# bytedance/DecompDiff

Measured on AMD Instinct MI355X. Metric: denoising steps/sec (1000-step reverse) per pocket, higher is better.
Workload: dtype f32

## Files before the change

### decompdiff_amd/csrc/dd_api.hip

```cpp
#include <mutex>
#include <thread>
#include <vector>
#include <stdlib.h>
#include <string.h>
#include <stdio.h>
#include <string>
#include <sys/stat.h>
#include <unistd.h>

#include "dd_kernels.hpp"

namespace dd {

struct Workspace {
  float *xa, *xb, *h, *hb, *ew, *P, *PL, *PB, *P2, *PL2, *PB2, *Ek, *Ev, *Rk, *Rv, *q1bl, *qn, *ql, *ql2, *qlnb, *qb, *A, *Anb, *dxe, *dxb, *ga, *gc, *gr, *h2, *hs;
  int32_t* nbr;
  int32_t* counters;
  size_t total;
};

static inline size_t align64(size_t n) { return (n + 63) & ~(size_t)63; }

static Workspace carve(float* base, int B, int NP, int NL, int K) {
  Workspace w;
  const size_t N = (size_t)NP + NL, Eb = (size_t)NL * (NL > 0 ? NL - 1 : 0);
  size_t off = 0;
  auto take = [&](size_t n) { float* p = base ? base + off : nullptr; off += align64(n); return p; };
  w.xa = take(B * N * 3);
  w.xb = take(B * N * 3);
  w.h = take(B * N * 128);
  w.hb = take(B * Eb * 128);
  w.nbr = reinterpret_cast<int32_t*>(take(B * N * K));
  w.ew = take(B * N * K);
  w.P = take(B * N * 640);
  w.PL = take((size_t)B * NL * 1280);
  w.PB = take(B * Eb * 640);
  w.P2 = take(B * N * 256);
  w.PL2 = take((size_t)B * NL * 1024);
  w.PB2 = take(B * Eb * 256);
  w.Ek = take(B * Eb * 128);
  w.Ev = take(B * Eb * 128);
  w.Rk = take(B * Eb * 128);
  w.Rv = take(B * Eb * 128);
  w.q1bl = take(B * Eb * 128);
  w.qn = take(B * N * 128);
  w.ql = take((size_t)B * NL * 128);
  w.ql2 = take((size_t)B * NL * 128);
  w.qlnb = take((size_t)B * NL * 128);
  w.qb = take(B * Eb * 128);
  w.A = take(B * N * 128);
  w.Anb = take((size_t)B * NL * 128);
  w.dxe = take((size_t)B * NL * 3);
  w.dxb = take((size_t)B * NL * 3);
  w.ga = take((size_t)B * NL * 3);
  w.gc = take((size_t)B * NL * 3);
  w.gr = take((size_t)B * NL * 3);
#if defined(DD_DEBUG_OPTIONS) && DD_DEBUG_OPTIONS
  w.h2 = take(B * N * 128);
  w.hs = take(B * N * 128);
#else
  w.h2 = w.hs = nullptr;
#endif
  w.counters = reinterpret_cast<int32_t*>(take(DD_NUM_COUNTERS + DD_NUM_FLAGS));
  w.total = off;
  return w;
}

static inline int num_v(const dd_sampler* s) { return s->num_v > 0 ? s->num_v : DD_NUM_V; }

static int check_shapes(const dd_sampler* s) {
  if (!s || !s->weights || !s->slot_off || !s->workspace) return DD_ERR_BAD_ARG;
  if (s->B <= 0 || s->NP < 0 || s->NL < 2 || s->K <= 0 || s->num_layers < 1 || s->num_layers > 64) return DD_ERR_BAD_ARG;
  const int N = s->NP + s->NL;
  if (s->NL > DD_NL_MAX || N > DD_N_MAX || s->K > DD_KNN_MAX || s->K > N - 1) return DD_ERR_UNSUPPORTED_SHAPE;
  if (s->num_v != 0 && s->num_v != 8 && s->num_v != 13 && s->num_v != 23) return DD_ERR_UNSUPPORTED_SHAPE;
  if (num_v(s) != DD_NUM_V && s->l0_tables != nullptr) return DD_ERR_BAD_ARG;
  if (s->workspace_floats < dd_workspace_floats(s->B, s->NP, s->NL, s->K)) return DD_ERR_WORKSPACE_TOO_SMALL;
  if ((s->nl_real != nullptr) != (s->bl_prefix != nullptr) || (s->np_real != nullptr && s->nl_real == nullptr)) return DD_ERR_BAD_ARG;
  return DD_OK;
}

struct Profiler {
  static constexpr int MAXEV = 512;
  hipEvent_t start[MAXEV], stop[MAXEV];
  int cat[MAXEV];
  int n = 0, created = 0;
};
static Profiler* g_prof = nullptr;

struct ProfScope {
  hipStream_t st; int idx;
  ProfScope(int cat, hipStream_t s) : st(s), idx(-1) {
    if (g_prof && g_prof->n < Profiler::MAXEV) {
      idx = g_prof->n++;
      g_prof->cat[idx] = cat;
      (void)hipEventRecord(g_prof->start[idx], st);
    }
  }
  ~ProfScope() { if (idx >= 0) (void)hipEventRecord(g_prof->stop[idx], st); }
};
#define DD_TRYP(cat, expr)               \
  do {                                  \
    ProfScope prof_scope__(cat, st);    \
    int rc__ = (expr);                  \
    if (rc__ != DD_OK) return rc__;     \
  } while (0)

#define DD_TRY(expr)            \
  do {                          \
    int rc__ = (expr);          \
    if (rc__ != DD_OK) return rc__; \
  } while (0)

extern int g_gemm_ksplit;
#if defined(DD_DEBUG_OPTIONS) && DD_DEBUG_OPTIONS
extern int g_tail_variant;
#endif
static bool g_gemm_ksplit_on() { return g_gemm_ksplit != 0; }
struct DevCtx {
  hipStream_t side = nullptr;
  hipEvent_t ev_qa_fork[8], ev_qb_fork[8], ev_fork[9], ev_join[9];
};
static DevCtx g_dev_ctx[16];
static std::mutex g_capture_mutex;
static DevCtx& dev_ctx() {
  int dev = 0;
  if (hipGetDevice(&dev) != hipSuccess || dev < 0 || dev >= 16) dev = 0;
  return g_dev_ctx[dev];
}
#define g_side (dev_ctx().side)
#define g_ev_qa_fork (dev_ctx().ev_qa_fork)
#define g_ev_qb_fork (dev_ctx().ev_qb_fork)
#define g_ev_fork (dev_ctx().ev_fork)
#define g_ev_join (dev_ctx().ev_join)
#ifndef DD_SIDE_LIN_DEFAULT
#define DD_SIDE_LIN_DEFAULT 0
#endif
#if defined(DD_DEBUG_OPTIONS) && DD_DEBUG_OPTIONS
#define DD_OPT static int
#else
#define DD_OPT static constexpr int
#endif
DD_OPT g_step_fused = 1;
DD_OPT g_step_fold = 1;
DD_OPT g_xup_in_asm = 1;
DD_OPT g_sched = 4;
DD_OPT g_xup_in_pos = 0;
DD_OPT g_fused_max_nl = DD_NL_MAX;
DD_OPT g_defer_pos = 0;
DD_OPT g_lin_with_pb2 = 1;
DD_OPT g_pb_early = 1;
DD_OPT g_q1_in_gemm = 1;
DD_OPT g_l0_tables = 1;
DD_OPT g_head_fused = 1;
DD_OPT g_side_lin = DD_SIDE_LIN_DEFAULT;
static int g_lin_in_node = [] { const char* e = getenv("DD_LIN_IN_NODE"); return e ? (e[0] == '1' ? 1 : (e[0] == '0' ? 0 : -1)) : -1; }();
static int g_lin_proj_main = [] { const char* e = getenv("DD_LIN_PROJ_MAIN"); return e ? (e[0] == '1' ? 1 : 0) : 0; }();
static bool lin_in_node_for(int B, int NL) {
  if (g_lin_in_node >= 0) return g_lin_in_node != 0;
  return (long)B * NL * (NL - 1) < 8L * 256 * 2;
}
DD_OPT g_head_rows_first = 0;
DD_OPT g_heads_early = 1;
DD_OPT g_q_in_pos = 1;
extern int g_pos_waves;
DD_OPT g_p2_in_pos = 0;
static int g_side_low_priority = [] { const char* e = getenv("DD_SIDE_PRIO"); return (e && e[0] == '1') ? 1 : ((e && e[0] == '2') ? 2 : 0); }();
static int g_overlap = 1;
static int ensure_side_stream() {
  if (g_side) return DD_OK;
  {
    int lo = 0, hi = 0;
    if (hipDeviceGetStreamPriorityRange(&lo, &hi) != hipSuccess) { lo = 0; (void)hipGetLastError(); }
    if (hipStreamCreateWithPriority(&g_side, hipStreamNonBlocking, g_side_low_priority == 1 ? lo : (g_side_low_priority == 2 ? hi : 0)) != hipSuccess) return DD_ERR_HIP;
  }
  for (int i = 0; i < 8; ++i)
    if (hipEventCreateWithFlags(&g_ev_qa_fork[i], hipEventDisableTiming) != hipSuccess ||
        hipEventCreateWithFlags(&g_ev_qb_fork[i], hipEventDisableTiming) != hipSuccess)
      return DD_ERR_HIP;
  for (int i = 0; i < 9; ++i)
    if (hipEventCreateWithFlags(&g_ev_fork[i], hipEventDisableTiming) != hipSuccess ||
        hipEventCreateWithFlags(&g_ev_join[i], hipEventDisableTiming) != hipSuccess)
      return DD_ERR_HIP;
  return DD_OK;
}

static int g_fuse = 1;
extern long long* g_gemm_dbg;
extern long long* g_node_trace;
static long long* g_dbg_clock = nullptr;
static int g_dbg_mode = -1;


static int attn_dispatch(int mode, const AttnArgs& a0, hipStream_t st) {
  AttnArgs a = a0;
  a.dbg_clock = (mode == g_dbg_mode) ? g_dbg_clock : nullptr;
  return launch_attn2(mode, a, st);
}

struct StepFold {
  bool advance = false;
  bool fold_tail = false;
  const float* xprev = nullptr;
};

__global__ __launch_bounds__(256) void k_bond_head_pre_att(const float* __restrict__ P, const float* __restrict__ x,
                                                           const float* __restrict__ dxe, const float* __restrict__ dxb, int NP, int NL,
                                                           const float* __restrict__ W_r, const float* __restrict__ b1,
                                                           const float* __restrict__ offset, float coeff,
                                                           const int32_t* __restrict__ nl_real, long rows, float* __restrict__ out) {
  constexpr int G = 20;
  const int lane = threadIdx.x & 63;
  const long nwaves = (long)gridDim.x * 4;
  float2 wr[G];
  float c[G];
#pragma unroll
  for (int k = 0; k < G; ++k) {
    wr[k] = *reinterpret_cast<const float2*>(W_r + k * 128 + 2 * lane);
    c[k] = offset[k];
  }
  const float2 bb = *reinterpret_cast<const float2*>(b1 + 2 * lane);
  const int N = NP + NL, NLm1 = NL - 1;
  const long Eb = (long)NL * NLm1;
  for (long e = (long)blockIdx.x * 4 + (threadIdx.x >> 6); e < rows; e += nwaves) {
    const int b = (int)(e / Eb);
    const int r = (int)(e - (long)b * Eb);
    const int t = r / NLm1, sp = r - t * NLm1;
    const int src = sp + (sp >= t);
    float2* o = reinterpret_cast<float2*>(out + e * 128 + 2 * lane);
    if (nl_real != nullptr && (t >= nl_real[b] || src >= nl_real[b])) {
      *o = make_float2(0.f, 0.f);
      continue;
    }
    float xd[3], xs[3];
#pragma unroll
    for (int q = 0; q < 3; ++q) {
      xd[q] = x[((long)b * N + NP + t) * 3 + q];
      xs[q] = x[((long)b * N + NP + src) * 3 + q];
      if (dxe != nullptr) {
        const long id = ((long)b * NL + t) * 3 + q, is = ((long)b * NL + src) * 3 + q;
// ... 208 lines not shown
      pe.B = B; pe.NP = NP; pe.NL = NL; pe.K = K; pe.x = xcur; pe.nbr = w.nbr; pe.ew = w.ew;
      pe.kd = w.PL2; pe.vd = w.PL2 + 128; pe.ld_kd = pe.ld_vd = 1024; pe.ks = w.P2; pe.vs = w.P2 + 128; pe.ld_ks = pe.ld_vs = 256;
      pe.q = w.ql; pe.Akp = LW(l, DD_PE_Akp); pe.Avp = LW(l, DD_PE_Avp); pe.lnk = LW(l, DD_PE_lnk); pe.lnv = LW(l, DD_PE_lnv);
      pe.W2k = LW(l, DD_PE_W2k); pe.W2v16 = LW(l, DD_PE_W2v); pe.b2v16 = LW(l, DD_PE_b2v); pe.out = w.dxe;
      pb.B = B; pb.NP = NP; pb.NL = NL; pb.K = K; pb.x = xcur;
      pb.kd = w.PL2 + 384; pb.ks = w.PL2 + 512; pb.vd = w.PL2 + 640; pb.vs = w.PL2 + 768; pb.ld_kd = pb.ld_ks = pb.ld_vd = pb.ld_vs = 1024;
      pb.ke = w.PB2; pb.ve = w.PB2 + 128; pb.ld_ke = pb.ld_ve = 256;
      pb.q = w.ql2; pb.lnk = LW(l, DD_PB_lnk); pb.lnv = LW(l, DD_PB_lnv);
      pb.W2k = LW(l, DD_PB_W2k); pb.W2v16 = LW(l, DD_PB_W2v); pb.b2v16 = LW(l, DD_PB_b2v); pb.out = w.dxb; pb.x_next = nullptr;
      pe.qhid = w.PL2 + 256; pe.ld_qhid = 1024; pe.lnq = LW(l, DD_PE_lnq); pe.W2q = LW(l, DD_PE_W2qT); pe.b2q = LW(l, DD_PE_b2q);
      pb.qhid = w.PL2 + 896; pb.ld_qhid = 1024; pb.lnq = LW(l, DD_PB_lnq); pb.W2q = LW(l, DD_PB_W2qT); pb.b2q = LW(l, DD_PB_b2q);
      if (two_streams) {
        if (hipEventRecord(g_ev_fork[l], st) != hipSuccess) return DD_ERR_HIP;
        DD_TRY(launch_gemm_tail(ta, st));
        if (hipStreamWaitEvent(g_side, g_ev_fork[l], 0) != hipSuccess) return DD_ERR_HIP;
        DD_TRY(launch_gemm_tail(tb, g_side));
        if (l + 1 == L && hipEventRecord(g_ev_join[l], g_side) != hipSuccess) return DD_ERR_HIP;
        DD_TRY(launch_attn2_pos(pe, pb, st));
      } else {
        DD_TRYP(DD_PROF_GEMM, launch_gemm_tail(ta, st));
        DD_TRYP(DD_PROF_GEMM, launch_gemm_tail(tb, st));
        DD_TRYP(DD_PROF_ATTN_PE, launch_attn2_pos(pe, pb, st));
      }
      if (l + 1 < L && ta.total + tb.total != total_mid) return DD_ERR_BAD_ARG;
      const bool deferred = l + 1 < L || (fold && fold->fold_tail);
      if (deferred) xup_prev = xcur;
      else DD_TRYP(DD_PROF_MISC, launch_xupdate(xcur, w.dxe, w.dxb, B, NP, NL, xnext, st));
    }
    float* t = xcur; xcur = xnext; xnext = t;
  }
  if (head_join && hipStreamWaitEvent(st, g_ev_join[8], 0) != hipSuccess) return DD_ERR_HIP;
  if (two_streams && hipStreamWaitEvent(st, g_ev_join[L - 1], 0) != hipSuccess) return DD_ERR_HIP;
  if (!s->pred_pos) return DD_ERR_BAD_ARG;
  if (xup_prev != nullptr) {
    fold->xprev = xup_prev;
    return DD_OK;
  }
  DD_TRYP(DD_PROF_MISC, launch_extract_ligand(xcur, B, NP, NL, s->pred_pos, st));
  return DD_OK;
}

#endif

static int check_node_out(const dd_node_out* no, const dd_sampler* s) {
  if (no == nullptr) return DD_OK;
  if (!s || no->num_layers != s->num_layers || no->num_layers < 1 || no->num_layers > 64) return DD_ERR_BAD_ARG;
  for (int l = 0; l < no->num_layers; ++l)
    if (!no->layer[l] || (reinterpret_cast<size_t>(no->layer[l]) & 15) != 0) return DD_ERR_BAD_ARG;
  return DD_OK;
}

static int forward_impl(const dd_sampler* s, hipStream_t st, StepFold* fold = nullptr, const dd_bond_head* bh = nullptr,
                        const dd_node_out* no = nullptr) {
  DD_TRY(check_shapes(s));
  DD_TRY(check_node_out(no, s));
  const bool pre_att = is_pre_att(bh);
  const bool out_fc = no != nullptr;
  const int B = s->B, NP = s->NP, NL = s->NL, K = s->K, N = NP + NL;
  const long Eb = (long)NL * (NL - 1);
  Workspace w = carve(s->workspace, B, NP, NL, K);
  const float* W = s->weights;
  const int64_t* off = s->slot_off;
  auto LW = [&](int l, int slot) { return W + off[(long)l * DD_NUM_LAYER_SLOTS + slot]; };
  auto GW = [&](int slot) { return W + off[(long)s->num_layers * DD_NUM_LAYER_SLOTS + slot]; };

  float* xcur = w.xa;
  float* xnext = w.xb;
  float* hcur = w.h;
  const long hN = (long)N * 128;
  const bool fused = g_fuse && NL <= g_fused_max_nl && g_dbg_clock == nullptr;
  const bool overlap = fused && g_overlap && g_prof == nullptr && s->num_layers <= 8;
#if defined(DD_DEBUG_OPTIONS) && DD_DEBUG_OPTIONS
  if (out_fc && (g_sched >= 5 || g_side_lin)) return DD_ERR_UNSUPPORTED_SHAPE;
  if (fused && !pre_att && g_sched >= 5 && s->num_layers <= DD_FLAG_LAYERS && g_q1_in_gemm && g_gemm_ksplit_on() && g_q_in_pos && g_head_fused &&
      g_xup_in_asm && !g_xup_in_pos)
    return forward_tail(s, st, fold, overlap);
#endif
  if (out_fc && !fused) return DD_ERR_UNSUPPORTED_SHAPE;
  if (overlap) DD_TRY(ensure_side_stream());

  const bool l0 = fused && g_l0_tables && g_q1_in_gemm && g_gemm_ksplit_on() && s->l0_tables && s->l0_P && s->l0_qn &&
                  s->nl_real == nullptr;
  int32_t* advance = (fold && fold->advance) ? s->step_counter : nullptr;
  bool head_join = false;
  if (overlap && g_head_fused) {
    auto head = [&](hipStream_t sx, int parts) -> int {
      return launch_head_all(s->protein_h, s->protein_pos, s->lig_pos, s->lig_v, s->lig_aux, GW(DD_G_W_lemb), GW(DD_G_b_lemb), B, NP, NL,
                             K, w.h, w.xa, w.xb, s->lig_bond, (long)B * Eb, GW(DD_G_W_bemb), GW(DD_G_b_bemb), w.hb, w.counters, advance,
                             w.nbr, w.ew, GW(DD_G_EW_W1T), GW(DD_G_EW_b1), GW(DD_G_EW_ln), GW(DD_G_EW_w2), GW(DD_G_EW_b2),
                             s->np_real, s->nl_real, l0 ? s->l0_tables : nullptr, s->l0_P, w.PL, s->l0_qn, w.qlnb, w.PB, w.qb, sx,
                             parts, num_v(s));
    };
    if (hipEventRecord(g_ev_fork[8], st) != hipSuccess || hipStreamWaitEvent(g_side, g_ev_fork[8], 0) != hipSuccess) return DD_ERR_HIP;
    if (g_head_rows_first) DD_TRYP(DD_PROF_MISC, head(st, 2));
    DD_TRYP(DD_PROF_MISC, head(g_side, 1));
    if (hipEventRecord(g_ev_join[8], g_side) != hipSuccess) return DD_ERR_HIP;
    head_join = true;
    if (!g_head_rows_first) DD_TRYP(DD_PROF_MISC, head(st, 2));
  } else {
    DD_TRYP(DD_PROF_MISC, launch_embed_all(s->protein_h, s->protein_pos, s->lig_pos, s->lig_v, s->lig_aux, GW(DD_G_W_lemb),
                                           GW(DD_G_b_lemb), B, NP, NL, w.h, w.xa, w.xb, s->lig_bond, (long)B * Eb, GW(DD_G_W_bemb),
                                           GW(DD_G_b_bemb), w.hb, w.counters, st, advance, num_v(s)));
    if (l0)
      DD_TRYP(DD_PROF_MISC, launch_layer0_rows(s->l0_tables, s->lig_v, s->lig_aux, s->lig_bond, B, NP, NL, s->l0_P, w.PL, s->l0_qn,
                                                w.qlnb, w.PB, w.qb, st));
    hipStream_t gs = st;
    if (overlap) {
      if (hipEventRecord(g_ev_fork[8], st) != hipSuccess || hipStreamWaitEvent(g_side, g_ev_fork[8], 0) != hipSuccess) return DD_ERR_HIP;
      gs = g_side;
    }
    DD_TRYP(DD_PROF_MISC, launch_knn(w.xa, B, N, K, w.nbr, gs, NP, s->np_real, s->nl_real));
    DD_TRYP(DD_PROF_MISC, launch_edge_weights(w.xa, w.nbr, B, N, K, GW(DD_G_EW_W1T), GW(DD_G_EW_b1), GW(DD_G_EW_ln), GW(DD_G_EW_w2),
                               GW(DD_G_EW_b2), w.ew, gs, NP, s->np_real, s->nl_real));
    if (overlap) {
      if (hipEventRecord(g_ev_join[8], g_side) != hipSuccess) return DD_ERR_HIP;
      head_join = true;
    }
  }
  int pending_join = -1;
  bool heads_done = false;
  struct DeferredPos { bool armed; AttnArgs pe, pb; float *xcur, *xnext; int layer; bool xup; } dpos;
  dpos.armed = false;
  auto flush_pos = [&]() -> int {
    if (!dpos.armed) return DD_OK;
    dpos.armed = false;
    if (hipStreamWaitEvent(g_side, g_ev_fork[dpos.layer], 0) != hipSuccess) return DD_ERR_HIP;
    int rc = launch_attn2_pos(dpos.pe, dpos.pb, g_side);
    if (rc == DD_OK && !dpos.xup) rc = launch_xupdate(dpos.xcur, w.dxe, w.dxb, B, NP, NL, dpos.xnext, g_side);
    if (rc != DD_OK) return rc;
    if (hipEventRecord(g_ev_join[dpos.layer], g_side) != hipSuccess) return DD_ERR_HIP;
    pending_join = dpos.layer;
    return DD_OK;
  };
  const float* xup_prev = nullptr;
  for (int l = 0; l < s->num_layers && fused; ++l) {
    const int nE = (int)(B * Eb);
    const bool lin_in_node = !out_fc && lin_in_node_for(B, NL) && g_lin_with_pb2 && !g_side_lin && g_heads_early;
    float* const anb_cur = (l & 1) ? w.A : w.Anb;
    const float* const anb_prev = (lin_in_node && l > 0) ? ((l & 1) ? w.Anb : w.A) : nullptr;
    auto add_anb = [&](GemmArgs& g, bool all_nodes) {
      g.X2 = anb_cur; g.x2_N = all_nodes ? N : NL; g.x2_NP = all_nodes ? NP : 0;
    };
    auto launch_batch1 = [&](int ll, hipStream_t sx) -> int {
      return launch_projections1(s, w, ll, hcur, w.P, sx, ll == l ? anb_prev : (lin_in_node ? anb_cur : nullptr));
    };
    auto launch_batch1_part = [&](int ll, int part, hipStream_t sx, const float* hsrc, const GemmArgs* lin_dup) -> int {
      if (part == 0) {
        GemmArgs j[2] = {gemm_args(w.hb, nE, 0, 128, nE, LW(ll, DD_W_b1), LW(ll, DD_b_b1), nullptr, w.PB, nE, 0, 640, 640, 0),
                         gemm_args(w.hb, nE, 0, 128, nE, LW(ll, DD_W_b1), LW(ll, DD_b_b1), nullptr, w.PB, nE, 0, 640, 640, 0)};
        if (lin_dup) { j[1] = j[0]; j[0] = *lin_dup; }
        return launch_gemm128_batch(j, lin_dup ? 2 : 1, sx);
      }
      GemmArgs j[2] = {
          gemm_args(hsrc, B * N, 0, 128, B * N, LW(ll, DD_W_n1), LW(ll, DD_b_n1), nullptr, w.P, B * N, 0, 640, 640, 0),
          gemm_args(hsrc + (long)NP * 128, NL, hN, 128, B * NL, LW(ll, DD_W_l1), LW(ll, DD_b_l1), nullptr, w.PL, B * NL, 0, 1280, 1280, 0)};
      if (lin_in_node) { add_anb(j[0], true); add_anb(j[1], false); }
      return launch_gemm128_batch(j, 2, sx);
    };
    const bool ahead = overlap && g_sched >= 1;
    const bool ahead_split = overlap && g_sched >= 2;
    const bool ahead_b2 = overlap && g_sched >= 3 && g_q1_in_gemm && g_gemm_ksplit_on();
    const bool two_joins = ahead_b2 && g_sched >= 4;
    const bool proj_main = lin_in_node && g_lin_proj_main && two_joins && ahead_split;
    const bool pb_early = g_pb_early && g_lin_with_pb2 && !ahead && !lin_in_node;
    const bool l0_here = l0 && l == 0;
    if (pb_early && l > 0) DD_TRYP(DD_PROF_GEMM, launch_batch1_part(l, 1, st, hcur, nullptr));
    else if (!(ahead && l > 0) && !l0_here) DD_TRYP(DD_PROF_GEMM, launch_batch1(l, st));
    const bool q1_in_gemm = g_q1_in_gemm && g_gemm_ksplit_on();
    auto launch_b2 = [&](int ll, hipStream_t sx) -> int {
      GemmArgs j[3] = {
          gemm_args(w.q1bl, nE, 0, 128, nE, LW(ll, DD_BL_W2q), LW(ll, DD_BL_b2q), LW(ll, DD_BL_lnq), w.qb, nE, 0, 128, 128, 0),
          gemm_args(w.P + 512, B * N, 0, 640, B * N, LW(ll, DD_NE_W2q), LW(ll, DD_NE_b2q), LW(ll, DD_NE_lnq), w.qn, B * N, 0, 128, 128, 0),
          gemm_args(w.PL + 512, B * NL, 0, 1280, B * NL, LW(ll, DD_NB_W2q), LW(ll, DD_NB_b2q), LW(ll, DD_NB_lnq), w.qlnb, B * NL, 0, 128, 128, 0)};
      if (q1_in_gemm) return launch_queries_q1(s, w, ll, w.P, w.qn, sx);
      return launch_gemm128_batch(j, 3, sx);
    };
    const bool b2_ahead = ahead_b2 && q1_in_gemm && l > 0;
    bool b1_joined = false;
    if (q1_in_gemm && !b2_ahead) {
      if (ahead && l > 0) {
        if (hipStreamWaitEvent(st, g_ev_join[l], 0) != hipSuccess) return DD_ERR_HIP;
        b1_joined = true;
      }
      if (!l0_here) DD_TRYP(DD_PROF_GEMM, launch_b2(l, st));
    }
    DD_TRY(flush_pos());
    if (pending_join >= 0) {
      if (hipStreamWaitEvent(st, g_ev_join[pending_join], 0) != hipSuccess) return DD_ERR_HIP;
      pending_join = -1;
    }
    const bool late_join = two_joins && b2_ahead && !b1_joined;
    if (ahead && l > 0 && !b1_joined && hipStreamWaitEvent(st, late_join ? g_ev_qb_fork[l] : g_ev_join[l], 0) != hipSuccess)
      return DD_ERR_HIP;
    DD_TRYP(DD_PROF_ASSEMBLE, launch_bl_assemble(xcur, w.PB, w.PL, LW(l, DD_BL_Wgp), B, NP, NL, w.Ek, w.Ev,
                                                  q1_in_gemm ? nullptr : w.q1bl, w.Rk, w.Rv, st, xup_prev, w.dxe, w.dxb,
                                                  xup_prev ? xcur : nullptr));
    xup_prev = nullptr;
    if (!q1_in_gemm) DD_TRYP(DD_PROF_GEMM, launch_b2(l, st));
    if (head_join) {
      if (hipStreamWaitEvent(st, g_ev_join[8], 0) != hipSuccess) return DD_ERR_HIP;
      head_join = false;
    }
    if (late_join && hipStreamWaitEvent(st, g_ev_join[l], 0) != hipSuccess) return DD_ERR_HIP;
    {
      AttnArgs ne, nb, bl;
      memset(&ne, 0, sizeof(ne)); memset(&nb, 0, sizeof(nb)); memset(&bl, 0, sizeof(bl));
      ne.np_real = nb.np_real = bl.np_real = s->np_real; ne.nl_real = nb.nl_real = bl.nl_real = s->nl_real;
      bl.bl_prefix = s->bl_prefix;
      ne.B = B; ne.NP = NP; ne.NL = NL; ne.K = K; ne.x = xcur; ne.nbr = w.nbr; ne.ew = w.ew;
      const float* Pn = l0_here ? s->l0_P : w.P;
      ne.kd = Pn; ne.ks = Pn + 128; ne.vd = Pn + 256; ne.vs = Pn + 384; ne.ld_kd = ne.ld_ks = ne.ld_vd = ne.ld_vs = 640;
      ne.q = l0_here ? s->l0_qn : w.qn; ne.Akp = LW(l, DD_NE_Akp); ne.Avp = LW(l, DD_NE_Avp); ne.lnk = LW(l, DD_NE_lnk); ne.lnv = LW(l, DD_NE_lnv);
      ne.W2k = LW(l, DD_NE_W2k); ne.W2v = LW(l, DD_NE_W2v); ne.b2v = LW(l, DD_NE_b2v); ne.out = w.A;
      ne.work_counter = (l < 32) ? w.counters + 128 + 2 * l : nullptr;
      nb.B = B; nb.NP = NP; nb.NL = NL; nb.K = K; nb.x = xcur;
      nb.kd = w.PL; nb.ks = w.PL + 128; nb.vd = w.PL + 256; nb.vs = w.PL + 384; nb.ld_kd = nb.ld_ks = nb.ld_vd = nb.ld_vs = 1280;
      nb.ke = w.PB; nb.ve = w.PB + 128; nb.ld_ke = nb.ld_ve = 640;
      nb.q = w.qlnb; nb.lnk = LW(l, DD_NB_lnk); nb.lnv = LW(l, DD_NB_lnv);
      nb.W2k = LW(l, DD_NB_W2k); nb.W2v = LW(l, DD_NB_W2v); nb.b2v = LW(l, DD_NB_b2v); nb.out = w.Anb; nb.out_assign = 1;
      if (lin_in_node) {
        ne.out = hcur; ne.lin_W = LW(l, DD_W_lin); ne.lin_b = LW(l, DD_b_lin); ne.lin_add = anb_prev;
        nb.out = anb_cur; nb.lin_W = LW(l, DD_W_lin);
      }
      bl.B = B; bl.NP = NP; bl.NL = NL; bl.K = K; bl.x = xcur;
      bl.ke = w.Ek; bl.ve = w.Ev; bl.ld_ke = bl.ld_ve = 128;
      bl.q = w.qb; bl.Wakp = LW(l, DD_BL_Wakp); bl.Wavp = LW(l, DD_BL_Wavp);
      bl.lnk = LW(l, DD_BL_lnk); bl.lnv = LW(l, DD_BL_lnv);
      bl.W2k = LW(l, DD_BL_W2k); bl.W2v = LW(l, DD_BL_W2v); bl.b2v = LW(l, DD_BL_b2v); bl.out = w.hb;
      bl.Rk = w.Rk; bl.Rv = w.Rv;
      bl.work_counter = (l < 64) ? w.counters + l : nullptr;
      DD_TRYP(DD_PROF_ATTN_BL, launch_attn2_node(ne, nb, bl, st));
    }
    if (ahead_split && l + 1 < s->num_layers && hipEventRecord(g_ev_qa_fork[l + 1], st) != hipSuccess) return DD_ERR_HIP;
    const bool side_lin = g_side_lin && ahead_split && ahead_b2 && l + 1 < s->num_layers;
    float* const hold = hcur;
    GemmArgs lin_dup;
    if (out_fc) {
      NodeOutArgs na{w.A, w.Anb, hcur, hcur, no->layer[l], B, NP, NL};
      DD_TRYP(DD_PROF_GEMM, launch_node_out_fc(na, st));
    } else if (!lin_in_node) {
      GemmArgs g = gemm_args(w.A, B * N, 0, 128, B * N, LW(l, DD_W_lin), LW(l, DD_b_lin), nullptr, hcur, B * N, 0, 128, 128, 1);
      g.X2 = w.Anb; g.x2_N = N; g.x2_NP = NP;
      if (side_lin) {
        float* hnew = (hcur == w.h) ? w.h2 : w.h;
        g.Y = hnew; g.acc_src = hold;
        lin_dup = g; lin_dup.Y = w.hs;
        hcur = hnew;
      } else if (hcur != w.h) {
        g.Y = w.h; g.acc_src = hold;
        hcur = w.h;
      }
      if (g_lin_with_pb2) {
        GemmArgs j[3] = {g, gemm_args(w.hb, nE, 0, 128, nE, LW(l, DD_W_b2), LW(l, DD_b_b2), nullptr, w.PB2, nE, 0, 256, 256, 0),
                         gemm_args(w.hb, nE, 0, 128, nE, LW(l, DD_W_b2), LW(l, DD_b_b2), nullptr, w.PB2, nE, 0, 256, 256, 0)};
        const bool more = pb_early && l + 1 < s->num_layers;
        if (more)
          j[2] = gemm_args(w.hb, nE, 0, 128, nE, LW(l + 1, DD_W_b1), LW(l + 1, DD_b_b1), nullptr, w.PB, nE, 0, 640, 640, 0);
        DD_TRYP(DD_PROF_GEMM, launch_gemm128_batch(j, more ? 3 : 2, st));
      } else {
        DD_TRYP(DD_PROF_GEMM, launch_gemm128(g, st));
      }
    }
    if (ahead && !side_lin && !proj_main && l + 1 < s->num_layers && hipEventRecord(g_ev_fork[l + 1], st) != hipSuccess) return DD_ERR_HIP;
    GemmArgs p2j[4] = {
        gemm_args(hcur, B * N, 0, 128, B * N, LW(l, DD_W_n2), LW(l, DD_b_n2), nullptr, w.P2, B * N, 0, 256, 256, 0),
        gemm_args(hcur + (long)NP * 128, NL, hN, 128, B * NL, LW(l, DD_W_l2), LW(l, DD_b_l2), nullptr, w.PL2, B * NL, 0, 1024, 1024, 0),
        gemm_args(w.hb, nE, 0, 128, nE, LW(l, DD_W_b2), LW(l, DD_b_b2), nullptr, w.PB2, nE, 0, 256, 256, 0),
        gemm_args(w.hb, nE, 0, 128, nE, LW(l, DD_W_b2), LW(l, DD_b_b2), nullptr, w.PB2, nE, 0, 256, 256, 0)};
    int p2n = g_lin_with_pb2 ? 2 : 3;
    GemmArgs p2x[6];
    if (g_heads_early && g_lin_with_pb2 && l + 1 == s->num_layers) {
      p2j[2] = gemm_args(w.hb, nE, 0, 128, nE, GW(DD_G_BH_W1), GW(DD_G_BH_b1), nullptr, w.qb, nE, 0, 128, 128, 0);
      if (pre_att)
        p2j[2] = gemm_args(hcur + (long)NP * 128, NL, hN, 128, B * NL, bh->W_p, nullptr, nullptr, w.P, B * NL, 0, 128, 128, 0);
      p2j[3] = gemm_args(hcur + (long)NP * 128, NL, hN, 128, B * NL, GW(DD_G_VH_W1), GW(DD_G_VH_b1), nullptr, w.qn, B * NL, 0, 128, 128, 0);
      p2n = 4;
      heads_done = true;
    }
    int p2xn = 0;
    if (lin_in_node) {
      p2x[p2xn++] = p2j[0]; add_anb(p2x[0], true);
      p2x[p2xn++] = p2j[1]; add_anb(p2x[1], false);
      p2x[p2xn++] = gemm_args(w.hb, nE, 0, 128, nE, LW(l, DD_W_b2), LW(l, DD_b_b2), nullptr, w.PB2, nE, 0, 256, 256, 0);
      if (p2n == 4) {
        p2x[p2xn] = p2j[2];
        if (pre_att) add_anb(p2x[p2xn], false);
        ++p2xn;
        p2x[p2xn] = p2j[3]; add_anb(p2x[p2xn], false); ++p2xn;
      }
      if (proj_main && l + 1 < s->num_layers) {
        p2x[p2xn] = gemm_args(hcur, B * N, 0, 128, B * N, LW(l + 1, DD_W_n1), LW(l + 1, DD_b_n1), nullptr, w.P, B * N, 0, 640, 640, 0);
        add_anb(p2x[p2xn], true); ++p2xn;
        p2x[p2xn] = gemm_args(hcur + (long)NP * 128, NL, hN, 128, B * NL, LW(l + 1, DD_W_l1), LW(l + 1, DD_b_l1), nullptr, w.PL, B * NL, 0, 1280, 1280, 0);
        add_anb(p2x[p2xn], false); ++p2xn;
      }
    }
    bool p2_in_pos = g_p2_in_pos && g_lin_with_pb2 && g_q_in_pos && !g_xup_in_pos && g_pos_waves == 4 && NL <= 65 && l < 64 &&
                     !(overlap && !ahead);
    if (out_fc) {
      p2_in_pos = false;
      p2x[p2xn++] = p2j[0];
      p2x[p2xn++] = p2j[1];
      p2x[p2xn++] = gemm_args(w.hb, nE, 0, 128, nE, LW(l, DD_W_b2), LW(l, DD_b_b2), nullptr, w.PB2, nE, 0, 256, 256, 0);
      if (p2n == 4) { p2x[p2xn++] = p2j[2]; p2x[p2xn++] = p2j[3]; }
      if (pb_early && g_lin_with_pb2 && l + 1 < s->num_layers)
        p2x[p2xn++] = gemm_args(w.hb, nE, 0, 128, nE, LW(l + 1, DD_W_b1), LW(l + 1, DD_b_b1), nullptr, w.PB, nE, 0, 640, 640, 0);
      DD_TRYP(DD_PROF_GEMM, launch_gemm128_batch(p2x, p2xn, st));
    } else if (lin_in_node) {
      p2_in_pos = false;
      DD_TRYP(DD_PROF_GEMM, launch_gemm128_batch(p2x, p2xn, st));
      if (proj_main && l + 1 < s->num_layers && hipEventRecord(g_ev_fork[l + 1], st) != hipSuccess) return DD_ERR_HIP;
    }
    else if (!p2_in_pos) DD_TRYP(DD_PROF_GEMM, launch_gemm128_batch(p2j, p2n, st));
    const bool q_in_pos = g_q_in_pos;
// ... 290 lines not shown

extern "C" const char* dd_status_string(int status) {
  switch (status) {
    case DD_OK: return "ok";
    case DD_ERR_BAD_ARG: return "bad argument (null pointer or non-positive size)";
    case DD_ERR_UNSUPPORTED_SHAPE: return "unsupported shape (NL > 128, N > 2048, K > 64 or K > N-1)";
    case DD_ERR_WORKSPACE_TOO_SMALL: return "workspace too small (see dd_workspace_floats)";
    case DD_ERR_HIP: return "HIP launch/runtime error";
  }
  return "unknown status";
}

extern "C" int dd_abi_version(void) { return 9; }
extern "C" int dd_build_flags(void) {
  int f = 0;
#if defined(DD_DEBUG_OPTIONS) && DD_DEBUG_OPTIONS
  f |= 1;
#endif
#if defined(DD_EXACT_MATH) && DD_EXACT_MATH
  f |= 2;
#endif
  return f;
}

extern "C" int dd_layer0_tables(const dd_sampler* m, float* tables, void* stream) {
  if (!m || !tables || !m->weights || !m->slot_off || !m->workspace || !m->lig_v || !m->lig_aux || !m->lig_bond || !m->lig_pos)
    return DD_ERR_BAD_ARG;
  if (m->B != 1 || m->NP != 0 || m->NL != 16) return DD_ERR_BAD_ARG;
  int rc = dd::check_shapes(m);
  if (rc != DD_OK) return rc;
  hipStream_t st = (hipStream_t)stream;
  dd::Workspace w = dd::carve(m->workspace, 1, 0, 16, m->K);
  const float* W = m->weights;
  auto GW = [&](int slot) { return W + m->slot_off[(long)m->num_layers * DD_NUM_LAYER_SLOTS + slot]; };
  rc = dd::launch_embed_all(m->protein_h, m->protein_pos, m->lig_pos, m->lig_v, m->lig_aux, GW(DD_G_W_lemb), GW(DD_G_b_lemb), 1, 0, 16,
                            w.h, w.xa, w.xb, m->lig_bond, 240, GW(DD_G_W_bemb), GW(DD_G_b_bemb), w.hb, w.counters, st, nullptr);
  if (rc != DD_OK) return rc;
  if ((rc = dd::launch_projections1(m, w, 0, w.h, w.P, st)) != DD_OK) return rc;
  if ((rc = dd::launch_queries_q1(m, w, 0, w.P, w.qn, st)) != DD_OK) return rc;
  auto cp = [&](float* dst, const float* src, size_t n) {
    return hipMemcpyAsync(dst, src, n * sizeof(float), hipMemcpyDeviceToDevice, st) == hipSuccess;
  };
  bool ok = cp(tables, w.P, 16 * 640) && cp(tables + 16 * 640, w.PL, 16 * 1280) && cp(tables + 16 * 640 + 16 * 1280, w.PB, 5 * 640);
  float* tq = tables + 16 * 640 + 16 * 1280 + 5 * 640;
  ok = ok && cp(tq, w.qn, 16 * 128) && cp(tq + 16 * 128, w.qlnb, 16 * 128);
  for (int c = 0; c < 16 && ok; ++c) ok = cp(tq + 32 * 128 + (size_t)c * 5 * 128, w.qb + (size_t)c * 15 * 128, 5 * 128);
  return ok ? DD_OK : DD_ERR_HIP;
}

extern "C" int dd_layer0_prepare(const dd_sampler* s, void* stream) {
  if (!s || !s->weights || !s->slot_off || !s->l0_P || !s->l0_qn) return DD_ERR_BAD_ARG;
  if (s->NP <= 0) return DD_OK;
  if (!s->protein_h) return DD_ERR_BAD_ARG;
  const int B = s->B, NP = s->NP, N = s->NP + s->NL;
  const float* W = s->weights;
  auto LW = [&](int l, int slot) { return W + s->slot_off[(long)l * DD_NUM_LAYER_SLOTS + slot]; };
  using dd::gemm_args;
  dd::GemmArgs g1 = gemm_args(s->protein_h, NP, (long)NP * 128, 128, B * NP, LW(0, DD_W_n1), LW(0, DD_b_n1), nullptr, s->l0_P, NP,
                              (long)N * 640, 640, 640, 0);
  int rc = dd::launch_gemm128_batch(&g1, 1, (hipStream_t)stream);
  if (rc != DD_OK) return rc;
  dd::GemmArgs g2 = gemm_args(s->l0_P + 512, NP, (long)N * 640, 640, B * NP, LW(0, DD_NE_W2q), LW(0, DD_NE_b2q), LW(0, DD_NE_lnq),
                              s->l0_qn, NP, (long)N * 128, 128, 128, 0);
  return dd::launch_gemm128_batch(&g2, 1, (hipStream_t)stream);
}

extern "C" int dd_sampler_reset(const dd_sampler* s, void* stream) {
  if (!s || !s->step_counter) return DD_ERR_BAD_ARG;
  if (s->t_start < 0 || s->t_start >= s->T) return DD_ERR_BAD_ARG;
  return dd::launch_reset_run_state(s->step_counter, s->t_start, s->seed, (hipStream_t)stream);
}

extern "C" size_t dd_workspace_floats(int B, int NP, int NL, int K) {
  if (B <= 0 || NP < 0 || NL <= 0 || K <= 0) return 0;
  return dd::carve(nullptr, B, NP, NL, K).total;
}

extern "C" int dd_workspace_view(const dd_sampler* s, dd_ws_view* out) {
  if (!s || !out || !s->workspace) return DD_ERR_BAD_ARG;
  dd::Workspace w = dd::carve(s->workspace, s->B, s->NP, s->NL, s->K);
  out->x = (s->num_layers & 1) ? w.xb : w.xa;
  out->h = w.h; out->hb = w.hb; out->ew = w.ew; out->A = w.A; out->nbr = w.nbr;
  out->Anb = (dd::g_fuse && s->NL <= dd::g_fused_max_nl) ? w.Anb : nullptr;
  out->lin_in_node = 0;
  if (out->Anb && dd::lin_in_node_for(s->B, s->NL) && dd::g_lin_with_pb2 && !dd::g_side_lin && dd::g_heads_early) {
    out->lin_in_node = 1;
    out->Anb = ((s->num_layers - 1) & 1) ? w.A : w.Anb;
    out->A = nullptr;
  }
  return DD_OK;
}

extern "C" int dd_forward(const dd_sampler* s, void* stream) { return dd_forward_ex(s, nullptr, stream); }

extern "C" int dd_forward_ex(const dd_sampler* s, const dd_bond_head* bh, void* stream) { return dd_forward_ex2(s, bh, nullptr, stream); }

extern "C" int dd_forward_ex2(const dd_sampler* s, const dd_bond_head* bh, const dd_node_out* no, void* stream) {
  hipStream_t st = (hipStream_t)stream;
  int rc = dd::check_bond_head(bh);
  if (rc != DD_OK) return rc;
  rc = dd::forward_impl(s, st, nullptr, bh, no);
  if (rc != DD_OK) return rc;
  if (!s->pred_pos || !s->pred_v || !s->pred_bond) return DD_ERR_BAD_ARG;
  dd::Workspace w = dd::carve(s->workspace, s->B, s->NP, s->NL, s->K);
  const float* W = s->weights;
  const int64_t* off = s->slot_off;
  auto GW = [&](int slot) { return W + off[(long)s->num_layers * DD_NUM_LAYER_SLOTS + slot]; };
  const int rows_v = s->B * s->NL;
  const long rows_b = (long)s->B * s->NL * (s->NL - 1);
  hipLaunchKernelGGL(dd::k_head_logits, dim3((rows_v + 3) / 4), dim3(256), 0, st, w.qn, GW(DD_G_VH_W2), GW(DD_G_VH_b2),
                     rows_v, dd::num_v(s), s->pred_v);
  hipLaunchKernelGGL(dd::k_head_logits, dim3((unsigned)((rows_b + 3) / 4)), dim3(256), 0, st, w.qb, GW(DD_G_BH_W2),
                     GW(DD_G_BH_b2), (int)rows_b, DD_NUM_B, s->pred_bond);
  DD_CHECK_LAUNCH();
  return DD_OK;
}

namespace dd {
extern int g_node_split_trial;
int node_split_lookup(int B, int NP, int NL, int K);
void node_split_store(int B, int NP, int NL, int K, int n_bl);
bool node_split_applies(int B, int NL, int n_cu);
}

static std::string node_split_cache_path(int n_cu) {
  const char* off = getenv("DD_NODE_SPLIT_CACHE");
  if (off && off[0] == '0') return std::string();
  std::string dir;
  if (const char* d = getenv("DD_NODE_SPLIT_CACHE_DIR")) dir = d;
  else if (const char* x = getenv("XDG_CACHE_HOME")) dir = std::string(x) + "/decompdiff_amd";
  else if (const char* h = getenv("HOME")) dir = std::string(h) + "/.cache/decompdiff_amd";
  else return std::string();
  int dev = 0;
  hipDeviceProp_t prop;
  if (hipGetDevice(&dev) != hipSuccess || hipGetDeviceProperties(&prop, dev) != hipSuccess) { (void)hipGetLastError(); return std::string(); }
  std::string name = std::string(prop.gcnArchName) + "_" + prop.name;
  for (char& c : name) if (!((c >= 'a' && c <= 'z') || (c >= 'A' && c <= 'Z') || (c >= '0' && c <= '9'))) c = '_';
  unsigned h = 2166136261u;
  for (const char* p = __DATE__ " " __TIME__; *p; ++p) h = (h ^ (unsigned char)*p) * 16777619u;
  char tag[64];
  snprintf(tag, sizeof(tag), "_cu%d_abi%d_%08x", n_cu, dd_abi_version(), h);
  return dir + "/node_split_" + name + tag + ".txt";
}
static int node_split_cache_read(const std::string& path, int B, int NP, int NL, int K) {
  if (path.empty()) return -1;
  FILE* f = fopen(path.c_str(), "r");
  if (!f) return -1;
  int b, np, nl, k, n, found = -1;
  while (fscanf(f, "%d %d %d %d %d", &b, &np, &nl, &k, &n) == 5)
    if (b == B && np == NP && nl == NL && k == K) found = n;
  fclose(f);
  return found;
}
static void node_split_cache_append(const std::string& path, int B, int NP, int NL, int K, int n_bl) {
  if (path.empty()) return;
  const size_t slash = path.rfind('/');
  if (slash != std::string::npos) {
    std::string dir = path.substr(0, slash);
    for (size_t i = 1; i <= dir.size(); ++i)
      if (i == dir.size() || dir[i] == '/') (void)mkdir(dir.substr(0, i).c_str(), 0755);
  }
  std::string all;
  if (FILE* f = fopen(path.c_str(), "r")) {
    char buf[256];
    while (fgets(buf, sizeof(buf), f)) all += buf;
    fclose(f);
  }
  char line[96];
  snprintf(line, sizeof(line), "%d %d %d %d %d\n", B, NP, NL, K, n_bl);
  all += line;
  char tmp[32];
  snprintf(tmp, sizeof(tmp), ".tmp%d", (int)getpid());
  const std::string t = path + tmp;
  FILE* f = fopen(t.c_str(), "w");
  if (!f) return;
  const bool ok = fwrite(all.data(), 1, all.size(), f) == all.size();
  fclose(f);
  if (!ok || rename(t.c_str(), path.c_str()) != 0) (void)unlink(t.c_str());
}

static int autotune_node_split(const dd_sampler* s, hipStream_t st) {
  static int n_cu = 0;
  if (n_cu == 0) {
    int dev = 0;
    hipDeviceProp_t prop;
    if (hipGetDevice(&dev) != hipSuccess || hipGetDeviceProperties(&prop, dev) != hipSuccess) return DD_ERR_HIP;
    n_cu = prop.multiProcessorCount > 0 ? prop.multiProcessorCount : 256;
  }
  const bool fused = dd::g_fuse && s->NL <= dd::g_fused_max_nl && dd::g_dbg_clock == nullptr;
  static const bool enabled = [] { const char* e = getenv("DD_NODE_SPLIT_AUTOTUNE"); return !(e && e[0] == '0'); }();
  if (!enabled) return DD_OK;
  if (!fused || !dd::node_split_applies(s->B, s->NL, n_cu) || dd::node_split_lookup(s->B, s->NP, s->NL, s->K) >= 0) return DD_OK;
  const std::string cache_path = node_split_cache_path(n_cu);
  {
    const int cached = node_split_cache_read(cache_path, s->B, s->NP, s->NL, s->K);
    if (cached == 0 || (cached >= 16 && cached <= n_cu - 16 && cached % 8 == 0)) {
      dd::node_split_store(s->B, s->NP, s->NL, s->K, cached);
      return DD_OK;
    }
  }
  hipEvent_t e0, e1;
  if (hipEventCreate(&e0) != hipSuccess || hipEventCreate(&e1) != hipSuccess) return DD_ERR_HIP;
  int rc = DD_OK;
  auto time_split = [&](int n_bl, float& best) {
    dd::g_node_split_trial = n_bl;
    best = 1e30f;
    for (int rep = 0; rep < 3 && rc == DD_OK; ++rep) {
      if (hipEventRecord(e0, st) != hipSuccess) { rc = DD_ERR_HIP; break; }
      rc = dd::forward_impl(s, st);
      if (rc != DD_OK) break;
      float ms = 0.f;
      if (hipEventRecord(e1, st) != hipSuccess || hipEventSynchronize(e1) != hipSuccess ||
          hipEventElapsedTime(&ms, e0, e1) != hipSuccess) { rc = DD_ERR_HIP; break; }
      if (rep > 0 && ms < best) best = ms;
    }
  };
  int best_n = 0;
  float best_t = 0.f, t = 0.f;
  const int tiles = (s->NL - 2 + 15) / 16;
  const double w_bl = ((double)s->B * s->NL * (s->NL - 1) / 8.0) * (0.1 + 0.35 * tiles);
  const double w_node = (double)s->B * ((s->NP + 7) / 8 + (s->NL + 7) / 8) + (double)s->B * s->NL / 8.0;
  const int centre = (int)(n_cu * w_bl / (w_bl + w_node)) / 8 * 8;
  struct Seen { int B, K, tiles, offset; };
  static std::vector<Seen> seen;
  static std::mutex seen_mutex;
  int predicted = -1;
  {
    std::lock_guard<std::mutex> lock(seen_mutex);
    for (const Seen& e : seen)
      if (e.B == s->B && e.K == s->K && e.tiles == tiles) predicted = centre + e.offset;
  }
  if (predicted >= 0) {
    predicted = predicted < 16 ? 16 : (predicted > n_cu - 16 ? n_cu - 16 : predicted);
    best_t = 1e30f;
    for (int n : {predicted, predicted - 8, predicted + 8}) {
      if (rc != DD_OK || n < 16 || n > n_cu - 16) continue;
      time_split(n, t);
      if (t < best_t) { best_t = t; best_n = n; }
    }
  } else {
    time_split(0, best_t);
    const int lo = centre - 32 < n_cu / 4 ? n_cu / 4 : centre - 32, hi = centre + 16 > n_cu - 16 ? n_cu - 16 : centre + 16;
    for (int n = lo; n <= hi && rc == DD_OK; n += 16) {
      time_split(n, t);
      if (t < best_t) { best_t = t; best_n = n; }
    }
    if (best_n > 0)
      for (int n : {best_n - 8, best_n + 8}) {
        if (rc != DD_OK || n < 16 || n > n_cu - 16) continue;
        time_split(n, t);
        if (t < best_t) { best_t = t; best_n = n; }
      }
    if (rc == DD_OK && best_n > 0) {
      std::lock_guard<std::mutex> lock(seen_mutex);
      seen.push_back(Seen{s->B, s->K, tiles, best_n - centre});
    }
  }
  dd::g_node_split_trial = -1;
  (void)hipEventDestroy(e0);
  (void)hipEventDestroy(e1);
  if (rc == DD_OK) {
    dd::node_split_store(s->B, s->NP, s->NL, s->K, best_n);
    node_split_cache_append(cache_path, s->B, s->NP, s->NL, s->K, best_n);
  }
  return rc;
}

extern "C" int dd_debug_node_split_cache_path(char* out, int cap) {
  if (!out || cap <= 0) return DD_ERR_BAD_ARG;
  int dev = 0;
  hipDeviceProp_t prop;
  if (hipGetDevice(&dev) != hipSuccess || hipGetDeviceProperties(&prop, dev) != hipSuccess) { (void)hipGetLastError(); return DD_ERR_HIP; }
  const std::string p = node_split_cache_path(prop.multiProcessorCount > 0 ? prop.multiProcessorCount : 256);
  if ((int)p.size() + 1 > cap) return DD_ERR_BAD_ARG;
  memcpy(out, p.c_str(), p.size() + 1);
  return DD_OK;
}

static int one_step(const dd_sampler* s, hipStream_t st, const dd_bond_head* bh = nullptr, const dd_node_out* no = nullptr) {
  dd::StepFold fold;
  fold.advance = fold.fold_tail = dd::g_step_fold != 0;
  int rc = dd::forward_impl(s, st, &fold, bh, no);
  if (rc != DD_OK) return rc;
  return dd::heads_and_step(s, st, &fold);
}

extern "C" int dd_reverse_step(const dd_sampler* s, const float* logits_v, const float* logits_b, const float* x0, void* stream) {
  if (!s || !logits_v || !logits_b || !x0 || !s->step_counter || !s->tab_pos || !s->tab_v || !s->tab_b || !s->atom_std ||
      !s->offset || !s->workspace)
    return DD_ERR_BAD_ARG;
  int rc = dd::check_shapes(s);
  if (rc != DD_OK) return rc;
  return dd::reverse_step_from_logits(s, logits_v, logits_b, x0, (hipStream_t)stream);
}

extern "C" int dd_sample_steps(const dd_sampler* s, int n_steps, void* stream) { return dd_sample_steps_ex(s, nullptr, n_steps, stream); }

extern "C" int dd_sample_steps_ex(const dd_sampler* s, const dd_bond_head* bh, int n_steps, void* stream) {
  return dd_sample_steps_ex2(s, bh, nullptr, n_steps, stream);
}

extern "C" int dd_sample_steps_ex2(const dd_sampler* s, const dd_bond_head* bh, const dd_node_out* no, int n_steps, void* stream) {
  if (dd::check_bond_head(bh) != DD_OK || dd::check_node_out(no, s) != DD_OK) return DD_ERR_BAD_ARG;
  if (!s || n_steps < 0 || !s->step_counter || !s->tab_pos || !s->tab_v || !s->tab_b || !s->atom_std || !s->offset ||
      !s->pred_pos)
    return DD_ERR_BAD_ARG;
  hipStream_t st = (hipStream_t)stream;
  for (int i = 0; i < n_steps; ++i) {
    int rc = one_step(s, st, bh, no);
    if (rc != DD_OK) return rc;
  }
  return DD_OK;
}

extern "C" int dd_sample_steps_graph(const dd_sampler* s, int n_steps, void* stream) {
  return dd_sample_steps_graph_ex(s, nullptr, n_steps, stream);
}

extern "C" int dd_sample_steps_graph_ex(const dd_sampler* s, const dd_bond_head* bh, int n_steps, void* stream) {
  return dd_sample_steps_graph_ex2(s, bh, nullptr, n_steps, stream);
}

extern "C" int dd_sample_steps_graph_ex2(const dd_sampler* s, const dd_bond_head* bh, const dd_node_out* no, int n_steps, void* stream) {
  if (dd::check_bond_head(bh) != DD_OK || dd::check_node_out(no, s) != DD_OK) return DD_ERR_BAD_ARG;
  if (!s || n_steps < 0 || !s->step_counter || !s->tab_pos || !s->tab_v || !s->tab_b || !s->atom_std || !s->offset ||
      !s->pred_pos)
    return DD_ERR_BAD_ARG;
  if (n_steps == 0) return DD_OK;
  hipStream_t st = (hipStream_t)stream;
  int rc = dd::check_shapes(s);
  if (rc != DD_OK) return rc;
  hipGraph_t graph = nullptr;
  hipGraphExec_t exec = nullptr;
  if (st == nullptr) return DD_ERR_BAD_ARG;
  rc = autotune_node_split(s, st);
  if (rc != DD_OK) return rc;
  std::unique_lock<std::mutex> capture_lock(dd::g_capture_mutex);
  if (hipStreamBeginCapture(st, hipStreamCaptureModeThreadLocal) != hipSuccess) {
    (void)hipGetLastError();
    return DD_ERR_HIP;
  }
  rc = one_step(s, st, bh, no);
  hipError_t e = hipStreamEndCapture(st, &graph);
  capture_lock.unlock();
  if (rc != DD_OK || e != hipSuccess || !graph) {
    if (graph) (void)hipGraphDestroy(graph);
// ... 132 lines not shown
      for (auto& t : th) t.join();
      for (int i = 0; i < n; ++i) if (trc[i] != DD_OK) rc = trc[i];
    } else {
      for (int k = 0; k < n_steps && rc == DD_OK; ++k)
        for (int i = 0; i < n; ++i)
          if (hipGraphLaunch(exec[i], (hipStream_t)streams[i]) != hipSuccess) { rc = DD_ERR_HIP; break; }
    }
  }
  for (int i = 0; i < n; ++i)
    if (hipStreamSynchronize((hipStream_t)streams[i]) != hipSuccess) rc = rc == DD_OK ? DD_ERR_HIP : rc;
  for (int i = n - 1; i >= 0; --i) {
    if (exec[i]) (void)hipGraphExecDestroy(exec[i]);
    if (graph[i]) (void)hipGraphDestroy(graph[i]);
  }
  if (rc != DD_OK) (void)hipGetLastError();
  return rc;
}

extern "C" int dd_profile_step(const dd_sampler* s, int n_iters, float* ms_per_category, void* stream) {
  if (!s || !ms_per_category || n_iters <= 0) return DD_ERR_BAD_ARG;
  hipStream_t st = (hipStream_t)stream;
  static dd::Profiler prof;
  if (!prof.created) {
    for (int i = 0; i < dd::Profiler::MAXEV; ++i) {
      if (hipEventCreate(&prof.start[i]) != hipSuccess || hipEventCreate(&prof.stop[i]) != hipSuccess) return DD_ERR_HIP;
    }
    prof.created = 1;
  }
  for (int c = 0; c < DD_NUM_PROF_CATS; ++c) ms_per_category[c] = 0.f;
  int rc = DD_OK;
  for (int it = 0; it < n_iters && rc == DD_OK; ++it) {
    prof.n = 0;
    dd::g_prof = &prof;
    rc = one_step(s, st);
    { dd::ProfScope empty_pair(DD_PROF_EVENT_PAIR, st); }
    dd::g_prof = nullptr;
    if (hipStreamSynchronize(st) != hipSuccess) return DD_ERR_HIP;
    for (int i = 0; i < prof.n; ++i) {
      float ms = 0.f;
      if (hipEventElapsedTime(&ms, prof.start[i], prof.stop[i]) != hipSuccess) return DD_ERR_HIP;
      ms_per_category[prof.cat[i]] += ms;
    }
  }
  for (int c = 0; c < DD_NUM_PROF_CATS; ++c) ms_per_category[c] /= (float)n_iters;
  return rc;
}

static int g_options_epoch = 0;
extern "C" int dd_debug_set_clock_buffer(long long* buf, int mode) {
  ++g_options_epoch;
  if (mode == 100) { dd::g_gemm_dbg = buf; return DD_OK; }
  if (mode == 200) { dd::g_node_trace = buf; return DD_OK; }
  dd::g_gemm_dbg = nullptr;
  dd::g_dbg_clock = buf;
  dd::g_dbg_mode = buf ? mode : -1;
  return DD_OK;
}

extern "C" int dd_debug_options_epoch(void) { return g_options_epoch; }

extern "C" int dd_debug_set_fusion(int mode) {
  ++g_options_epoch;
  if (mode != 0 && mode != 1 && mode != 3) return DD_ERR_BAD_ARG;
  dd::g_fuse = (mode == 1 || mode == 3) ? 1 : 0;
  dd::g_overlap = mode == 1 ? 1 : 0;
  return DD_OK;
}

namespace dd { extern int g_pos_g_mode; extern int g_gemm_ksplit; extern int g_attn_waves; extern int g_attn_persist; extern int g_pos_waves; extern int g_bl_first; extern int g_gemm_xcd; }
#if defined(DD_DEBUG_OPTIONS) && DD_DEBUG_OPTIONS
extern "C" int dd_queue_error(const dd_sampler* s, void* stream, int* code) {
  if (!s || !s->workspace || !code) return DD_ERR_BAD_ARG;
  dd::Workspace w = dd::carve(s->workspace, s->B, s->NP, s->NL, s->K);
  int32_t v = 0;
  if (hipMemcpyAsync(&v, w.counters + dd::DD_NUM_COUNTERS + dd::DD_FLAG_ERR, sizeof(v), hipMemcpyDeviceToHost, (hipStream_t)stream) != hipSuccess ||
      hipStreamSynchronize((hipStream_t)stream) != hipSuccess)
    return DD_ERR_HIP;
  *code = (int)v;
  if (v != 0 && hipMemsetAsync(w.counters + dd::DD_NUM_COUNTERS + dd::DD_FLAG_ERR, 0, sizeof(v), (hipStream_t)stream) != hipSuccess) return DD_ERR_HIP;
  return DD_OK;
}
#endif

extern "C" int dd_debug_node_split(int B, int NP, int NL, int K) { return dd::node_split_lookup(B, NP, NL, K); }

extern "C" int dd_debug_schedule(void) { return dd::g_p2_in_pos ? 1 : 0; }

extern "C" int dd_debug_set_option(int key, int value) {
  ++g_options_epoch;
  if (key == 0) return dd_debug_set_fusion(value);
#if defined(DD_DEBUG_OPTIONS) && DD_DEBUG_OPTIONS
  if (key == 1) { dd::g_gemm_ksplit = value ? 1 : 0; return DD_OK; }
  if (key == 3) { dd::g_attn_persist = value ? 1 : 0; return DD_OK; }
  if (key == 24) { dd::g_head_fused = value ? 1 : 0; return DD_OK; }
  if (key == 22) { dd::g_l0_tables = value ? 1 : 0; return DD_OK; }
  if (key == 21) { dd::g_gemm_xcd = value ? 1 : 0; return DD_OK; }
  if (key == 20) { dd::g_step_fold = value ? 1 : 0; return DD_OK; }
  if (key == 19) { dd::g_xup_in_asm = value ? 1 : 0; return DD_OK; }
  if (key == 18) { if (value < 0 || value > 1024) return DD_ERR_BAD_ARG; dd::g_bl_first = value; return DD_OK; }
  if (key == 17) { dd::g_pb_early = value ? 1 : 0; return DD_OK; }
  if (key == 16) { dd::g_lin_with_pb2 = value ? 1 : 0; return DD_OK; }
  if (key == 14) { dd::g_defer_pos = value ? 1 : 0; return DD_OK; }
  if (key == 13) { dd::g_fused_max_nl = value; return DD_OK; }
  if (key == 12) { dd::g_q1_in_gemm = value ? 1 : 0; return DD_OK; }
  if (key == 11) { dd::g_xup_in_pos = value ? 1 : 0; return DD_OK; }
  if (key == 9) { dd::g_q_in_pos = value ? 1 : 0; return DD_OK; }
  if (key == 8) { if (value < 0 || value > 5) return DD_ERR_BAD_ARG; dd::g_sched = value; return DD_OK; }
  if (key == 25) { dd::g_tail_variant = value; return DD_OK; }
  if (key == 27) { dd::g_side_lin = value ? 1 : 0; return DD_OK; }
  if (key == 30) { dd::g_p2_in_pos = value ? 1 : 0; return DD_OK; }
  if (key == 31) { dd::g_pos_g_mode = value & 3; return DD_OK; }
  if (key == 28) { dd::g_heads_early = value ? 1 : 0; return DD_OK; }
  if (key == 32) { dd::g_lin_in_node = value < 0 ? -1 : (value ? 1 : 0); return DD_OK; }
  if (key == 29) { dd::g_head_rows_first = value ? 1 : 0; return DD_OK; }
  if (key == 7) { dd::g_step_fused = value ? 1 : 0; return DD_OK; }
  if (key == 5) { if (value != 2 && value != 4 && value != 8) return DD_ERR_BAD_ARG; dd::g_pos_waves = value; return DD_OK; }
  if (key == 2) { if (value != 8) return DD_ERR_BAD_ARG; dd::g_attn_waves = value; return DD_OK; }
  return DD_ERR_BAD_ARG;
#else
  (void)value;
  return DD_ERR_BAD_ARG;
#endif
}
```

### decompdiff_amd/csrc/dd_attention2.hip

```cpp
#include <vector>
#include <type_traits>

#include "dd_kernels.hpp"
#include "dd_gemm_tile.hpp"

#ifndef DD_LN_FOLD
#define DD_LN_FOLD 1
#endif
#ifndef DD_FAST_ANGLE
#define DD_FAST_ANGLE 1
#endif
#ifndef DD_TRIP_SYNC
#define DD_TRIP_SYNC 6
#endif
static_assert(DD_TRIP_SYNC >= 1 && DD_TRIP_SYNC <= 7, "DD_TRIP_SYNC: the eight trip slots of the persistent workgroups allow 1 ... 7");
#ifndef DD_NODE_TRACE
#define DD_NODE_TRACE 0
#endif

namespace dd {

typedef float f32x4 __attribute__((ext_vector_type(4)));

namespace v2 {
// ... 154 lines not shown
  float p = -4.0544654832e-03f;
  p = fmaf(p, u, 2.1862573855e-02f);
  p = fmaf(p, u, -5.5911747027e-02f);
  p = fmaf(p, u, 9.6421528094e-02f);
  p = fmaf(p, u, -1.3908611309e-01f);
  p = fmaf(p, u, 1.9946561855e-01f);
  p = fmaf(p, u, -3.3329860447e-01f);
  p = fmaf(p, u, 9.9999933550e-01f);
  const float phi = p * x;
  const bool acute = c1 >= 0.f;
  const float th = acute ? 2.0f * phi : fmaf(-2.0f, phi, 3.14159265358979f);
  const float big = __builtin_amdgcn_sqrtf(0.5f * den);
  const float small = 0.5f * s1 * __builtin_amdgcn_rcpf(big);
  const float sh = acute ? small : big, ch = acute ? big : small;
  const float a6 = th * (1.0f / 6.0f), z = a6 * a6;
  const float ps = fmaf(fmaf(fmaf(-1.9515295891e-4f, z, 8.3321608736e-3f), z, -1.6666654611e-1f) * z, a6, a6);
  const float pc = fmaf(fmaf(fmaf(2.443315711809948e-5f, z, -1.388731625493765e-3f), z, 4.166664568298827e-2f) * z, z,
                        fmaf(-0.5f, z, 1.0f));
  const float st = 2.0f * ps * pc, ct = fmaf(-2.0f * ps, ps, 1.0f);
#else
  const float n = sqrtf(nn);
  const float th = atan2f(n, dt);
  const float n2 = fmaf(n, n, dt * dt);
  const float r = n2 > 0.f ? dd_rsqrt(n2) : 0.f;
  const float s1 = n * r, c1 = n2 > 0.f ? dt * r : 1.0f;
  const float s2 = 2.0f * s1 * c1, c2 = fmaf(c1, c1, -s1 * s1);
  const float s3 = fmaf(s2, c1, c2 * s1), c3 = fmaf(c2, c1, -s2 * s1);
  float sh, ch;
  if (c1 >= 0.f) { ch = sqrtf(0.5f * (1.0f + c1)); sh = 0.5f * s1 / ch; }
  else           { sh = sqrtf(0.5f * (1.0f - c1)); ch = 0.5f * s1 / sh; }
  float st, ct;
  sincos_small(th * (1.0f / 3.0f), st, ct);
#endif
  out[0] = cg == 0 ? th : (cg == 1 ? s1 : (cg == 2 ? s2 : s3));
  out[1] = cg == 0 ? sh : (cg == 1 ? st : (cg == 2 ? c1 : c2));
  out[2] = cg == 0 ? c3 : (cg == 1 ? ch : (cg == 2 ? ct : 0.f));
}

template <bool TR>
__device__ __forceinline__ void mfma_table_step(f32x4 (&acc)[8], const float* __restrict__ tb , float f) {
  const float4 w0 = *reinterpret_cast<const float4*>(tb);
  const float4 w1 = *reinterpret_cast<const float4*>(tb + 64);
  const float w[8] = {w0.x, w0.y, w0.z, w0.w, w1.x, w1.y, w1.z, w1.w};
#pragma unroll
  for (int nt = 0; nt < 8; ++nt)
    acc[nt] = TR ? __builtin_amdgcn_mfma_f32_16x16x4f32(f, w[nt], acc[nt], 0, 0, 0)
                 : __builtin_amdgcn_mfma_f32_16x16x4f32(w[nt], f, acc[nt], 0, 0, 0);
}

template <int MODE>
struct Lds {
  static constexpr bool TRIP = (MODE == M_BL);
  static constexpr bool KNN = (MODE == M_NE || MODE == M_PE);
  static constexpr bool RES = (MODE == M_NB || MODE == M_BL);
  static constexpr int WV = RES ? WB_FLOATS : 0;
  static constexpr int XPAD = KNN ? 128 : 0;
  static constexpr int TAB = WB_FLOATS + XPAD;
  static constexpr int LNP = WB_FLOATS * (RES ? 2 : 1) + XPAD + (KNN ? 4 * TABP : 0);
  static constexpr int WAO = LNP + 512;
  static constexpr int TOTAL = WAO + (TRIP ? 2 * 12 * 128 : 0);
};

__device__ __forceinline__ void pos_wait_tiles(const int32_t* counter, int target_in) {
  const bool fast = target_in < 0;
  const int target = fast ? -target_in : target_in;
  if (threadIdx.x == 0) {
    unsigned spins = 0;
    while (__hip_atomic_load(counter, __ATOMIC_RELAXED, __HIP_MEMORY_SCOPE_AGENT) < target) {
      if (spins == 0 || fast) __builtin_amdgcn_s_sleep(8);
      else if (spins == 1) __builtin_amdgcn_s_sleep(16);
      else if (spins == 2) __builtin_amdgcn_s_sleep(32);
      else if (spins == 3) __builtin_amdgcn_s_sleep(64);
      else __builtin_amdgcn_s_sleep(127);
      if (++spins > (1u << 20)) __builtin_trap();
    }
    __builtin_amdgcn_fence(__ATOMIC_ACQUIRE, "agent");
  }
  __syncthreads();
}

__host__ __device__ inline int ne_blocks_per_sample(int NP, int NL, int NW) { return (NP + NW - 1) / NW + (NL + NW - 1) / NW; }

template <int MODE, int MAXT, int NW, bool PERSIST = false, bool RAG = false, bool PAIR = false, bool STAMPS = true, bool WIDE = false,
          typename ARGS = AttnArgs>
__device__ __forceinline__ void attn2_body(const ARGS& a, const int block, float* smem) {
  constexpr bool KNN = (MODE == M_NE || MODE == M_PE);
  constexpr bool POS = (MODE == M_PE || MODE == M_PB);
  constexpr bool TRIP = (MODE == M_BL);
  constexpr bool BOND = (MODE == M_NB || MODE == M_PB);
  static_assert(!PAIR || (POS && !PERSIST), "wave pairs: coordinate modes");
  constexpr int NT = (PAIR ? 2 : 1) * NW * 64;
  using L = Lds<MODE>;
  constexpr int LNP = L::LNP, WAO = L::WAO;
  constexpr bool RES = L::RES;
  static_assert(!PERSIST || RES, "persistent workgroups need both weight images resident");
  float* WB = smem;
  float* WV = smem + L::WV;
  const int wave = PAIR ? ((threadIdx.x >> 6) % NW) : (threadIdx.x >> 6), lane0 = threadIdx.x & 63;
  const int role = PAIR ? ((threadIdx.x >> 6) / NW) : 0;
  const bool kside = !PAIR || role == 0, vside = !PAIR || role == 1;

  const int N = a.NP + a.NL, NLm1 = a.NL - 1, Eb = a.NL * NLm1;
  constexpr bool COMPACT = RAG && TRIP && PERSIST;
  const int nseg = COMPACT ? a.bl_prefix[a.B] : ((MODE == M_NE) ? a.B * N : (TRIP ? a.B * Eb : a.B * a.NL));
  int M = KNN ? a.K : (TRIP ? a.NL - 2 : NLm1);
  int T = (M + 15) >> 4;
  auto bl_dense_seg = [&](int r) -> int {
    if (!COMPACT) return r;
    int bb = 0;
    while (a.bl_prefix[bb + 1] <= r) ++bb;
    const int nm1 = a.nl_real[bb] - 1, e = r - a.bl_prefix[bb];
    return bb * Eb + (e / nm1) * NLm1 + (e % nm1);
  };
  const int ne_bps = ne_blocks_per_sample(a.NP, a.NL, NW), ne_nbp = (a.NP + NW - 1) / NW;
  const int ne_b = block / ne_bps, ne_rb = block % ne_bps;
  const bool wg_protein = (MODE == M_NE) && ne_rb < ne_nbp;
  if (MODE == M_NE && RAG && ne_b < a.B) {
    const int first = wg_protein ? ne_rb * NW : (ne_rb - ne_nbp) * NW;
    if (first >= (wg_protein ? (a.np_real ? a.np_real[ne_b] : a.NP) : a.nl_real[ne_b])) return;
  }
  long long* dbg = (STAMPS && a.dbg_clock) ? a.dbg_clock + (long)block * 16 : nullptr;
#define DD_STAMP(i) do { if (dbg && threadIdx.x == 0) dbg[i] = (long long)__builtin_amdgcn_s_memtime(); } while (0)
  DD_STAMP(0);

  auto stage_all = [&]() {
    stage_w2k_permuted<NT>(WB, a.W2k);
    if (RES) stage_w2k_permuted<NT>(WV, a.W2v);
    if (threadIdx.x < 64) {
      reinterpret_cast<float4*>(smem + LNP)[threadIdx.x] = reinterpret_cast<const float4*>(a.lnk)[threadIdx.x];
      reinterpret_cast<float4*>(smem + LNP + 256)[threadIdx.x] = reinterpret_cast<const float4*>(a.lnv)[threadIdx.x];
    }
    if (TRIP) {
      for (int i = threadIdx.x; i < 12 * 32; i += NT) {
        reinterpret_cast<float4*>(smem + WAO)[i] = reinterpret_cast<const float4*>(a.Wakp)[i];
        reinterpret_cast<float4*>(smem + WAO + 12 * 128)[i] = reinterpret_cast<const float4*>(a.Wavp)[i];
      }
    }
    if (KNN) {
      const int tyl = wg_protein ? 1 : 0;
      constexpr int PER = (4 * 768) / NT;
      static_assert((4 * 768) % NT == 0, "table staging assumes NT | 3072");
      float4 tmp[PER];
#pragma unroll
      for (int k = 0; k < PER; ++k) {
        const int i = threadIdx.x + k * NT, q = i / 768, w = i - q * 768;
        const float* src = (q < 2 ? a.Akp : a.Avp) + (tyl + 2 * (q & 1)) * TABP;
        tmp[k] = reinterpret_cast<const float4*>(src)[w];
      }
#pragma unroll
      for (int k = 0; k < PER; ++k) reinterpret_cast<float4*>(smem + L::TAB)[threadIdx.x + k * NT] = tmp[k];
    }
    __syncthreads();
  };
  int* sb = reinterpret_cast<int*>(smem + L::TOTAL);
  int it = 0;
  float4 qn0 = make_float4(0.f, 0.f, 0.f, 0.f), qn1 = qn0;
  auto trip_range = [&](int tr, int& base, int& cnt) {
    if (tr < a.trip_full) { base = tr * NW; cnt = NW; }
    else { base = a.trip_full * NW + (tr - a.trip_full) * a.trip_q; cnt = a.trip_q; }
    cnt = nseg - base < cnt ? nseg - base : cnt;
  };
  if (PERSIST) {
    if (threadIdx.x == 0) { sb[0] = atomicAdd(a.work_counter, 1); sb[8] = 0; }
    stage_all();
  }

  for (;;) {
  int lane = lane0;
  asm volatile("" : "+v"(lane) :: "memory");
  const int mm = lane & 15, cg = lane >> 4;
  int seg;
  if (PERSIST) {
    if (it > 0 && it % DD_TRIP_SYNC == 0) __syncthreads();
    int base, cnt;
    trip_range(__builtin_amdgcn_readfirstlane(sb[it & 7]), base, cnt);
    if (cnt <= 0) break;
    if (threadIdx.x == 0) {
      sb[(it + 1) & 7] = atomicAdd(a.work_counter, 1);
      __hip_atomic_store(&sb[8], it + 1, __ATOMIC_RELEASE, __HIP_MEMORY_SCOPE_WORKGROUP);
    }
    seg = wave < cnt ? bl_dense_seg(base + wave) : a.B * Eb;
  } else if (MODE == M_NE) {
    const int nd = wg_protein ? ne_rb * NW + wave : a.NP + (ne_rb - ne_nbp) * NW + wave;
    seg = (nd < (wg_protein ? a.NP : N) && ne_b < a.B) ? ne_b * N + nd : nseg;
  } else {
    seg = block * NW + wave;
  }
  bool active = seg < ((MODE == M_NE) ? a.B * N : (TRIP ? a.B * Eb : a.B * a.NL));

  int b = 0, si = 0, sj = 0, node = 0;
  if (active) {
    if (MODE == M_NE) { b = seg / N; node = seg % N; }
    else if (TRIP) { b = seg / Eb; const int e = seg % Eb; si = e / NLm1; const int jp = e % NLm1; sj = jp + (jp >= si ? 1 : 0); }
    else { b = seg / a.NL; si = seg % a.NL; node = a.NP + si; }
    if (RAG) {
      const int nlb = a.nl_real[b], npb = a.np_real ? a.np_real[b] : a.NP;
      if (MODE == M_NE) active = node < a.NP ? node < npb : node - a.NP < nlb;
      else if (TRIP) active = si < nlb && sj < nlb;
      else active = si < nlb;
      if (!KNN) { M = TRIP ? nlb - 2 : nlb - 1; T = (M + 15) >> 4; }
    }
  }
  const float* xb = a.x + (long)b * N * 3;
  const float* xl = xb + (long)a.NP * 3;
  const long nrow = (long)b * N + node;
  const long src_base = KNN ? (long)b * N : (long)b * a.NL;
  const long erow0 = (long)seg * NLm1;
  const long drow = (MODE == M_NE) ? (long)seg : (long)b * a.NL + si;
  const int tlo = si < sj ? si : sj, thi = si < sj ? sj : si;
  auto trip_k = [&](int mc) { int k = mc; if (k >= tlo) ++k; if (k >= thi) ++k; return k; };

  int jm[MAXT];
  int jT[MAXT][4];
  float dm[MAXT], ewm[MAXT][4];
  if (KNN && active) {
#pragma unroll
    for (int t = 0; t < MAXT; ++t) {
      const int m = 16 * t + mm;
      jm[t] = a.nbr[nrow * a.K + (m < M ? m : M - 1)];
#pragma unroll
      for (int r = 0; r < 4; ++r) {
        const int mr = 16 * t + 4 * cg + r;
        ewm[t][r] = a.ew[nrow * a.K + (mr < M ? mr : 0)];
        jT[t][r] = a.nbr[nrow * a.K + (mr < M ? mr : M - 1)];
      }
    }
    const float cx = xb[3 * node], cy = xb[3 * node + 1], cz = xb[3 * node + 2];
#pragma unroll
    for (int t = 0; t < MAXT; ++t) {
      const float rx = cx - xb[3 * jm[t]], ry = cy - xb[3 * jm[t] + 1], rz = cz - xb[3 * jm[t] + 2];
      dm[t] = sqrtf(rx * rx + ry * ry + rz * rz);
    }
  }

  if (!PERSIST) stage_all();
#if defined(DD_DEBUG_OPTIONS) && DD_DEBUG_OPTIONS
  if (POS && a.wait_flags != nullptr) {
    pos_wait_tiles(a.wait_flags + a.wait_idx, a.wait_n);
  }
#endif
  DD_STAMP(1);

  float4 q0 = make_float4(0.f, 0.f, 0.f, 0.f), q1 = q0;
  if (PERSIST && it > 0) {
    q0 = qn0; q1 = qn1;
  } else if (POS && a.W2q != nullptr && kside) {
    float* sc = smem + L::TOTAL + wave * 256;
    if (active) {
      float2 hv = *reinterpret_cast<const float2*>(a.qhid + drow * a.ld_qhid + 2 * lane);
      ln_relu2(hv.x, hv.y, a.lnq[2 * lane], a.lnq[2 * lane + 1], a.lnq[128 + 2 * lane], a.lnq[128 + 2 * lane + 1]);
      *reinterpret_cast<float2*>(sc + 2 * lane) = hv;
    }
    __builtin_amdgcn_fence(__ATOMIC_RELEASE, "wavefront");
    __builtin_amdgcn_wave_barrier();
    __builtin_amdgcn_fence(__ATOMIC_ACQUIRE, "wavefront");
    if (active) {
      const float2* wT = reinterpret_cast<const float2*>(a.W2q) + lane;
      float a0 = 0.f, a1 = 0.f;
#pragma unroll 4
      for (int k4 = 0; k4 < 32; ++k4) {
        const float4 z = *reinterpret_cast<const float4*>(sc + 4 * k4);
        const float2 u0 = wT[(4 * k4 + 0) * 64], u1 = wT[(4 * k4 + 1) * 64], u2 = wT[(4 * k4 + 2) * 64], u3 = wT[(4 * k4 + 3) * 64];
        a0 = fmaf(u0.x, z.x, a0); a1 = fmaf(u0.y, z.x, a1);
        a0 = fmaf(u1.x, z.y, a0); a1 = fmaf(u1.y, z.y, a1);
        a0 = fmaf(u2.x, z.z, a0); a1 = fmaf(u2.y, z.z, a1);
        a0 = fmaf(u3.x, z.w, a0); a1 = fmaf(u3.y, z.w, a1);
// ... 344 lines not shown
        if (t < T) {
          const f32x4 V = Vt[t];
#pragma unroll
          for (int r = 0; r < 4; ++r) {
            const int m = 16 * t + 4 * cg + r;
            const int mc = m < M ? m : 0;
            int j;
            const float* xs;
            if (KNN) { j = jT[t][r]; xs = xb; }
            else { j = mc + (mc >= si ? 1 : 0); xs = xl; }
            const int ii = KNN ? node : si;
            const float coef = S[t][r] * (V[r] + bv);
            dx = fmaf(coef, xs[3 * ii] - xs[3 * j], dx);
            dy = fmaf(coef, xs[3 * ii + 1] - xs[3 * j + 1], dy);
            dz = fmaf(coef, xs[3 * ii + 2] - xs[3 * j + 2], dz);
          }
        }
      }
      dx = wave_sum(dx) * (1.0f / 16.0f);
      dy = wave_sum(dy) * (1.0f / 16.0f);
      dz = wave_sum(dz) * (1.0f / 16.0f);
    }
    if (active && vside) {
      if (lane < 3) {
        const float v = lane == 0 ? dx : (lane == 1 ? dy : dz);
        if (MODE == M_PE || a.x_next == nullptr) {
          a.out[(long)seg * 3 + lane] = v;
        } else {
          const long xi = ((long)b * N + node) * 3 + lane;
          a.x_next[xi] = a.x[xi] + a.dxe[(long)seg * 3 + lane] + v;
        }
      }
    }
    DD_STAMP(10);
    return;
  }

  f32x4 Z[8];
#pragma unroll
  for (int nt = 0; nt < 8; ++nt) Z[nt] = f32x4{0.f, 0.f, 0.f, 0.f};
  if (active) {
#pragma unroll
    for (int t = 0; t < MAXT; ++t) {
      if (t < T) {
        float Tz[32];
        finish_T(t, Tz);
#pragma unroll
        for (int ks = 0; ks < 4; ++ks)
#pragma unroll
          for (int nt = 0; nt < 8; ++nt)
            Z[nt] = __builtin_amdgcn_mfma_f32_16x16x4f32(Tz[4 * nt + ks], S[t][ks], Z[nt], 0, 0, 0);
      }
    }
  }
  DD_STAMP(8);

  DD_STAMP(9);
  if (PERSIST) {
    while (__hip_atomic_load(&sb[8], __ATOMIC_ACQUIRE, __HIP_MEMORY_SCOPE_WORKGROUP) < it + 1) {}
    int base2, cnt2;
    trip_range(sb[(it + 1) & 7], base2, cnt2);
    if (wave < cnt2) {
      const int nseg2 = bl_dense_seg(base2 + wave);
      qn0 = *reinterpret_cast<const float4*>(a.q + (long)nseg2 * 128 + mm * 8);
      qn1 = *reinterpret_cast<const float4*>(a.q + (long)nseg2 * 128 + mm * 8 + 4);
    }
  }
  constexpr bool LIN = (MODE == M_NE || MODE == M_NB) && !PERSIST;
  const bool lin = LIN && a.lin_W != nullptr;
  float4 Bw[8];
  float lin_old[4] = {0.f, 0.f, 0.f, 0.f};
  long lin_off[4] = {-1, -1, -1, -1};
  if (lin) {
    const float* bw = a.lin_W + (16 * wave + mm) * 128 + 4 * cg;
#pragma unroll
    for (int nt = 0; nt < 8; ++nt) Bw[nt] = *reinterpret_cast<const float4*>(bw + 16 * nt);
    if (cg < 2) {
      const int col = 16 * wave + mm;
      const float bias = (MODE == M_NE) ? a.lin_b[col] : 0.f;
#pragma unroll
      for (int r = 0; r < 4; ++r) {
        const int i = 4 * cg + r;
        if (MODE == M_NE) {
          const int nd = wg_protein ? ne_rb * NW + i : a.NP + (ne_rb - ne_nbp) * NW + i;
          bool ok = nd < (wg_protein ? a.NP : N) && ne_b < a.B;
          if (RAG && ok) ok = nd < a.NP ? nd < (a.np_real ? a.np_real[ne_b] : a.NP) : nd - a.NP < a.nl_real[ne_b];
          if (ok) {
            lin_off[r] = ((long)ne_b * N + nd) * 128 + col;
            float v = a.out[lin_off[r]];
            if (nd >= a.NP && a.lin_add != nullptr) v += a.lin_add[((long)ne_b * a.NL + nd - a.NP) * 128 + col];
            lin_old[r] = v + bias;
          }
        } else {
          const int sg = block * NW + i;
          bool ok = sg < a.B * a.NL;
          if (RAG && ok) ok = sg % a.NL < a.nl_real[sg / a.NL];
          if (ok) lin_off[r] = (long)sg * 128 + col;
        }
      }
    }
  }
  float* const lin_rows = smem + L::TOTAL + 16;
  if constexpr (NECO) {
    constexpr int XSTR = 16 * WPITCH + 16;
    float* const XB = smem;
    float* const SS = lin_rows + NW * WPITCH;
    float4 Bv[8];
    {
      const float* bv = a.W2v + (16 * wave + mm) * 128 + 4 * cg;
#pragma unroll
      for (int nt = 0; nt < 8; ++nt) Bv[nt] = *reinterpret_cast<const float4*>(bv + 16 * nt);
    }
    const int eh = mm >> 3;
    const float bias2 = a.b2v[16 * wave + mm];
    if (active) {
#pragma unroll
      for (int nt = 0; nt < 8; ++nt)
        *reinterpret_cast<float4*>(XB + wave * XSTR + mm * WPITCH + 16 * nt + 4 * cg) = make_float4(Z[nt][0], Z[nt][1], Z[nt][2], Z[nt][3]);
      if (cg == 0) SS[wave * 16 + mm] = ssum;
    }
    __syncthreads();
    const float* ar = XB + (mm >> 1) * XSTR + (2 * wave + (mm & 1)) * WPITCH + 4 * cg;
    f32x4 d0 = {0.f, 0.f, 0.f, 0.f}, d1 = {0.f, 0.f, 0.f, 0.f};
#pragma unroll
    for (int nt = 0; nt < 8; nt += 2) {
      const float4 a0 = *reinterpret_cast<const float4*>(ar + 16 * nt), a1 = *reinterpret_cast<const float4*>(ar + 16 * nt + 16);
      d0 = __builtin_amdgcn_mfma_f32_16x16x4f32(a0.x, Bv[nt].x, d0, 0, 0, 0);
      d1 = __builtin_amdgcn_mfma_f32_16x16x4f32(a1.x, Bv[nt + 1].x, d1, 0, 0, 0);
      d0 = __builtin_amdgcn_mfma_f32_16x16x4f32(a0.y, Bv[nt].y, d0, 0, 0, 0);
      d1 = __builtin_amdgcn_mfma_f32_16x16x4f32(a1.y, Bv[nt + 1].y, d1, 0, 0, 0);
      d0 = __builtin_amdgcn_mfma_f32_16x16x4f32(a0.z, Bv[nt].z, d0, 0, 0, 0);
      d1 = __builtin_amdgcn_mfma_f32_16x16x4f32(a1.z, Bv[nt + 1].z, d1, 0, 0, 0);
      d0 = __builtin_amdgcn_mfma_f32_16x16x4f32(a0.w, Bv[nt].w, d0, 0, 0, 0);
      d1 = __builtin_amdgcn_mfma_f32_16x16x4f32(a1.w, Bv[nt + 1].w, d1, 0, 0, 0);
    }
    const f32x4 d = d0 + d1;
#pragma unroll
    for (int u = 0; u < 2; ++u) {
      const int sI = 2 * cg + u;
      const int nd = wg_protein ? ne_rb * NW + sI : a.NP + (ne_rb - ne_nbp) * NW + sI;
      bool ok = nd < (wg_protein ? a.NP : N) && ne_b < a.B;
      if (RAG && ok) ok = nd < a.NP ? nd < (a.np_real ? a.np_real[ne_b] : a.NP) : nd - a.NP < a.nl_real[ne_b];
      const float val = fmaf(bias2, SS[sI * 16 + 2 * wave + eh], eh ? d[2 * u + 1] : d[2 * u]);
      if (lin) lin_rows[sI * WPITCH + 16 * wave + mm] = val;
      else if (ok) a.out[((long)ne_b * N + nd) * 128 + 16 * wave + mm] = val;
    }
  } else
  if (active) {
    float o[8];
#pragma unroll
    for (int j = 0; j < 8; ++j) {
      const float* wr = WV + (j * 16 + mm) * WPITCH + 4 * cg;
      float acc0 = 0.f, acc1 = 0.f;
#pragma unroll
      for (int nt = 0; nt < 8; nt += 2) {
        const float4 w0 = *reinterpret_cast<const float4*>(wr + 16 * nt);
        const float4 w1 = *reinterpret_cast<const float4*>(wr + 16 * nt + 16);
        acc0 = fmaf(w0.x, Z[nt][0], acc0); acc0 = fmaf(w0.y, Z[nt][1], acc0);
        acc0 = fmaf(w0.z, Z[nt][2], acc0); acc0 = fmaf(w0.w, Z[nt][3], acc0);
        acc1 = fmaf(w1.x, Z[nt + 1][0], acc1); acc1 = fmaf(w1.y, Z[nt + 1][1], acc1);
        acc1 = fmaf(w1.z, Z[nt + 1][2], acc1); acc1 = fmaf(w1.w, Z[nt + 1][3], acc1);
      }
      o[j] = acc0 + acc1;
      __builtin_amdgcn_sched_barrier(0);
    }
    const float p0 = swap16_sum(o[0], o[1]), p1 = swap16_sum(o[2], o[3]);
    const float p2 = swap16_sum(o[4], o[5]), p3 = swap16_sum(o[6], o[7]);
    float q0 = swap32_sum(p0, p1), q1 = swap32_sum(p2, p3);
    q0 = fmaf(a.b2v[mm * 8 + cg], ssum, q0);
    q1 = fmaf(a.b2v[mm * 8 + 4 + cg], ssum, q1);
    const bool nb_assign = (MODE == M_NB) && a.out_assign;
    if (lin) {
      lin_rows[wave * WPITCH + mm * 8 + cg] = q0;
      lin_rows[wave * WPITCH + mm * 8 + 4 + cg] = q1;
    } else {
      float* dst;
      if (MODE == M_NB && !nb_assign) dst = a.out + ((long)b * N + node) * 128 + mm * 8 + cg;
      else dst = a.out + (long)seg * 128 + mm * 8 + cg;
      if (MODE == M_NE || nb_assign) {
        dst[0] = q0; dst[4] = q1;
      } else {
        dst[0] += q0; dst[4] += q1;
      }
    }
  }
  if constexpr (LIN) {
    if (lin) {
      __syncthreads();
      const float* ar = lin_rows + (mm & 7) * WPITCH + 4 * cg;
      f32x4 d0 = {0.f, 0.f, 0.f, 0.f}, d1 = {0.f, 0.f, 0.f, 0.f};
#pragma unroll
      for (int nt = 0; nt < 8; nt += 2) {
        const float4 a0 = *reinterpret_cast<const float4*>(ar + 16 * nt), a1 = *reinterpret_cast<const float4*>(ar + 16 * nt + 16);
        d0 = __builtin_amdgcn_mfma_f32_16x16x4f32(a0.x, Bw[nt].x, d0, 0, 0, 0);
        d1 = __builtin_amdgcn_mfma_f32_16x16x4f32(a1.x, Bw[nt + 1].x, d1, 0, 0, 0);
        d0 = __builtin_amdgcn_mfma_f32_16x16x4f32(a0.y, Bw[nt].y, d0, 0, 0, 0);
        d1 = __builtin_amdgcn_mfma_f32_16x16x4f32(a1.y, Bw[nt + 1].y, d1, 0, 0, 0);
        d0 = __builtin_amdgcn_mfma_f32_16x16x4f32(a0.z, Bw[nt].z, d0, 0, 0, 0);
        d1 = __builtin_amdgcn_mfma_f32_16x16x4f32(a1.z, Bw[nt + 1].z, d1, 0, 0, 0);
        d0 = __builtin_amdgcn_mfma_f32_16x16x4f32(a0.w, Bw[nt].w, d0, 0, 0, 0);
        d1 = __builtin_amdgcn_mfma_f32_16x16x4f32(a1.w, Bw[nt + 1].w, d1, 0, 0, 0);
      }
      const f32x4 d = d0 + d1;
      if (cg < 2) {
#pragma unroll
        for (int r = 0; r < 4; ++r)
          if (lin_off[r] >= 0) a.out[lin_off[r]] = (MODE == M_NE) ? lin_old[r] + d[r] : d[r];
      }
    }
  }
  DD_STAMP(10);
  if (!PERSIST) break;
  ++it;
  }
#undef DD_STAMP
}

template <int MODE, int MAXT, int NW, bool RAG = false>
__global__ __launch_bounds__(NW * 64) void k_attn2(const AttnArgs a) {
  __shared__ __attribute__((aligned(16))) float smem[Lds<MODE>::TOTAL + ((MODE == M_PE || MODE == M_PB) ? NW * 256 : 0) +
                                                     ((MODE == M_NE || MODE == M_NB) ? NW * WPITCH + 16 + 128 : 0)];
  attn2_body<MODE, MAXT, NW, false, RAG>(a, blockIdx.x, smem);
}

constexpr int imax(int a, int b) { return a > b ? a : b; }

template <int MAXT, int NW, bool RAG = false, int KT = 2>
__global__ __launch_bounds__(NW * 64) void k_attn2_node(const AttnArgs ne, const AttnArgs nb, const AttnArgs bl, int n_ne, int n_nb,
                                                        int persist, int n_bl_first, const int32_t* wflags, int widx, int wn, int nep) {
  constexpr int SZ = imax(imax(Lds<M_NE>::TOTAL, Lds<M_NB>::TOTAL), Lds<M_BL>::TOTAL) + 12;
  __shared__ __attribute__((aligned(16))) float smem[SZ];
  int blk = blockIdx.x;
#if !DD_NODE_TRACE
  dd_wait_flags(wflags, widx, wn, -1, 0, DD_FLAG_ERR, 500);
#endif
  typedef const __attribute__((address_space(4))) AttnArgs KArgs;
  auto args = [](unsigned k) -> KArgs& {
    unsigned off = k * (unsigned)sizeof(AttnArgs);
    asm volatile("" : "+s"(off));
    return *reinterpret_cast<KArgs*>((const __attribute__((address_space(4))) char*)__builtin_amdgcn_kernarg_segment_ptr() + off);
  };
  static_assert(sizeof(AttnArgs) % 8 == 0, "kernel parameter layout");
  (void)ne; (void)nb; (void)bl; (void)nep;
#if DD_NODE_TRACE
  long long* const trace = (wn == -12345) ? reinterpret_cast<long long*>(const_cast<int32_t*>(wflags)) + (long)blockIdx.x * 16 : nullptr;
#define DD_TRACE_ST(i, v) __hip_atomic_store(trace + (i), (long long)(v), __ATOMIC_RELAXED, __HIP_MEMORY_SCOPE_SYSTEM)
  if (trace && threadIdx.x == 0) {
    DD_TRACE_ST(0, __builtin_amdgcn_s_memrealtime());
    DD_TRACE_ST(3, (long long)(unsigned)__builtin_amdgcn_s_getreg((31 << 11) | 4 ) |
                       ((long long)(unsigned)__builtin_amdgcn_s_getreg((3 << 11) | 20 ) << 32));
  }
#define DD_TRACE_END(kind) do { if (trace && threadIdx.x == 0) { DD_TRACE_ST(1, __builtin_amdgcn_s_memrealtime()); DD_TRACE_ST(2, kind); } } while (0)
#else
#define DD_TRACE_END(kind) do { } while (0)
#endif
  if (n_bl_first > 0) {
    if (blk < n_bl_first) {
      attn2_body<M_BL, MAXT, NW, true, RAG, false, false, (KT > 2)>(args(2), blk, smem);
      DD_TRACE_END(2);
      return;
    }
    blk -= n_bl_first;
    if (blk < n_ne) { attn2_body<M_NE, KT, NW, false, RAG, false, false, (KT > 2)>(args(0), blk, smem); DD_TRACE_END(0); }
    else { attn2_body<M_NB, MAXT, NW, false, RAG, false, false, (KT > 2)>(args(1), blk - n_ne, smem); DD_TRACE_END(1); }
    return;
  }
  if (blk < n_ne) attn2_body<M_NE, KT, NW, false, RAG, false, false, (KT > 2)>(args(0), blk, smem);
  else if (blk < n_ne + n_nb) attn2_body<M_NB, MAXT, NW, false, RAG, false, false, (KT > 2)>(args(1), blk - n_ne, smem);
  else if (persist) attn2_body<M_BL, MAXT, NW, true, RAG, false, false, (KT > 2)>(args(2), blk - n_ne - n_nb, smem);
  else attn2_body<M_BL, MAXT, NW, false, RAG, false, false, (KT > 2)>(args(2), blk - n_ne - n_nb, smem);
}
template <int MAXT, int NW, bool RAG = false, int KT = 2>
__global__ __launch_bounds__(NW * 128) void k_attn2_pos(const AttnArgs pe, const AttnArgs pb, int n_pe) {
  constexpr int SZ = imax(Lds<M_PE>::TOTAL, Lds<M_PB>::TOTAL) + NW * 256 + NW * imax(MAXT, KT) * 256;
  __shared__ __attribute__((aligned(16))) float smem[SZ];
  const int blk = blockIdx.x;
  dd_wait_flags(pe.wait_flags, pe.wait_idx, pe.wait_n, -1, 0, DD_FLAG_ERR, 400);
  if (blk < n_pe) attn2_body<M_PE, KT, NW, false, RAG, true, false, (KT > 2)>(pe, blk, smem);
  else attn2_body<M_PB, MAXT, NW, false, RAG, true, false, (KT > 2)>(pb, blk - n_pe, smem);
  if (pe.work_counter == nullptr) return;
  __shared__ int s_last;
  __syncthreads();
  if (threadIdx.x == 0) {
    __threadfence();
    s_last = atomicAdd(pe.work_counter, 1) == (int)gridDim.x - 1 ? 1 : 0;
  }
  __syncthreads();
  if (s_last) {
    __threadfence();
    const int n = pe.B * pe.NL * 3, N = pe.NP + pe.NL;
    const volatile float* dxe = pe.out;
    const volatile float* dxb = pb.out;
    for (int idx = threadIdx.x; idx < n; idx += NW * 128) {
      const int b = idx / (pe.NL * 3), r = idx % (pe.NL * 3);
      const long xi = ((long)b * N + pe.NP) * 3 + r;
      pe.x_next[xi] = pe.x[xi] + dxe[idx] + dxb[idx];
    }
    if (threadIdx.x == 0) *pe.work_counter = 0;
  }
}

#if defined(DD_DEBUG_OPTIONS) && DD_DEBUG_OPTIONS
struct PosGemm { GemmArgs job[4]; int end[4]; int nbx[4]; int njobs; int mode; };

__device__ __forceinline__ void pos_gemm_tiles(const PosGemm& pg, int first, int limit, float* smem) {
  const int half = __builtin_amdgcn_readfirstlane((int)(threadIdx.x >> 8));
  int tile = first + half;
  const bool valid = tile < limit;
  if (!valid) tile = first;
  int j = 0, base = 0;
#pragma unroll
  for (int i = 0; i < 3; ++i)
    if (j == i && tile >= pg.end[i] && i + 1 < pg.njobs) { base = pg.end[i]; j = i + 1; }
  j = __builtin_amdgcn_readfirstlane(j);
  const GemmArgs a = pg.job[j];
  const int lb = tile - base, nbx = pg.nbx[j];
  const int bx = valid ? lb % nbx : (1 << 20), by = lb / nbx;
  if (pg.mode & 1) gemm_tile_ksplit<false, false>(a, bx, by, smem + half * (2 * GT * GPH));
  else gemm_tile_ksplit<false, true>(a, bx, by, smem + half * (2 * GT * GPH));
}

template <int MAXT, int NW, bool RAG = false>
__global__ __launch_bounds__(NW * 128) void k_attn2_pos_g(const AttnArgs pe, const AttnArgs pb, int n_pe, const PosGemm pg, int n_g0,
                                                          int n_tiles0, int n_att, int n_tiles_all, int32_t* counter) {
  static_assert(NW == 4, "two 256-thread tile groups per workgroup");
  constexpr int SZ = imax(Lds<M_PE>::TOTAL, Lds<M_PB>::TOTAL) + NW * 256 + NW * MAXT * 256;
  static_assert(SZ >= 2 * 2 * GT * GPH, "two K-half tile images fit the attention workgroup's LDS");
  __shared__ __attribute__((aligned(16))) float smem[SZ];
  int blk = blockIdx.x;
  if (blk < n_g0 || blk >= n_g0 + n_att) {
    const bool lead = blk < n_g0;
    const int first = lead ? 2 * blk : n_tiles0 + 2 * (blk - n_g0 - n_att);
    pos_gemm_tiles(pg, first, lead ? n_tiles0 : n_tiles_all, smem);
    if (lead) {
      asm volatile("s_waitcnt vmcnt(0)" ::: "memory");
      __syncthreads();
      if (threadIdx.x == 0) {
        const int n_done = n_tiles0 - first < 2 ? n_tiles0 - first : 2;
        if (pg.mode & 1) __hip_atomic_fetch_add(counter, n_done, __ATOMIC_RELEASE, __HIP_MEMORY_SCOPE_AGENT);
        else __hip_atomic_fetch_add(counter, n_done, __ATOMIC_RELAXED, __HIP_MEMORY_SCOPE_AGENT);
      }
    }
    return;
  }
  blk -= n_g0;
  if (blk < n_pe) attn2_body<M_PE, 2, NW, false, RAG, true, false>(pe, blk, smem);
  else attn2_body<M_PB, MAXT, NW, false, RAG, true, false>(pb, blk - n_pe, smem);
}

#endif

#ifdef DD_ASM_ONLY
template __global__ void k_attn2_node<2, 8, false>(const AttnArgs, const AttnArgs, const AttnArgs, int, int, int, int, const int32_t*, int, int, int);
template __global__ void k_attn2_pos<2, 4, false>(const AttnArgs, const AttnArgs, int);
}
}
#else
template <int MODE, int MAXT, int NW>
static int launch_mode(const AttnArgs& a, int nseg, hipStream_t st) {
  if (nseg <= 0) return DD_OK;
  if (a.nl_real != nullptr) hipLaunchKernelGGL((k_attn2<MODE, MAXT, NW, true>), dim3((nseg + NW - 1) / NW), dim3(NW * 64), 0, st, a);
  else hipLaunchKernelGGL((k_attn2<MODE, MAXT, NW>), dim3((nseg + NW - 1) / NW), dim3(NW * 64), 0, st, a);
  DD_CHECK_LAUNCH();
  return DD_OK;
}

}

}
extern "C" int dd_weights_form(void) { return DD_LN_FOLD ? 1 : 0; }
namespace dd {

int g_attn_waves = 8;
int g_attn_persist = 1;
int g_bl_first = 1;
int g_node_split_trial = -1;
long long* g_node_trace = nullptr;
namespace {
struct NodeSplit { int B, NP, NL, K, n_bl; };
std::vector<NodeSplit> g_node_splits;
}
int node_split_lookup(int B, int NP, int NL, int K) {
  for (const NodeSplit& e : g_node_splits)
    if (e.B == B && e.NP == NP && e.NL == NL && e.K == K) return e.n_bl;
  return -1;
}
void node_split_store(int B, int NP, int NL, int K, int n_bl) {
  for (NodeSplit& e : g_node_splits)
    if (e.B == B && e.NP == NP && e.NL == NL && e.K == K) { e.n_bl = n_bl; return; }
  g_node_splits.push_back(NodeSplit{B, NP, NL, K, n_bl});
}
bool node_split_applies(int B, int NL, int n_cu) {
  return g_attn_persist && g_bl_first == 1 && (B * NL * (NL - 1) + 7) / 8 >= n_cu;
}

int launch_attn2(int mode, const AttnArgs& a, hipStream_t st) {
  using namespace v2;
  const int N = a.NP + a.NL;
  const bool small = a.NL <= 33;
  const bool big = a.NL > 65;
  if (a.NL > 129 || a.K > DD_KNN_MAX) return DD_ERR_UNSUPPORTED_SHAPE;
  switch (mode) {
    case M_NE: {
      const int nseg = a.B * v2::ne_blocks_per_sample(a.NP, a.NL, 8) * 8;
      return a.K <= 32 ? launch_mode<M_NE, 2, 8>(a, nseg, st) : launch_mode<M_NE, 4, 8>(a, nseg, st);
    }
    case M_PE: return a.K <= 32 ? launch_mode<M_PE, 2, 8>(a, a.B * a.NL, st) : launch_mode<M_PE, 4, 8>(a, a.B * a.NL, st);
    case M_NB: return small ? launch_mode<M_NB, 2, 8>(a, a.B * a.NL, st)
                            : (big ? launch_mode<M_NB, 8, 8>(a, a.B * a.NL, st) : launch_mode<M_NB, 4, 8>(a, a.B * a.NL, st));
    case M_PB: return small ? launch_mode<M_PB, 2, 8>(a, a.B * a.NL, st)
                            : (big ? launch_mode<M_PB, 8, 8>(a, a.B * a.NL, st) : launch_mode<M_PB, 4, 8>(a, a.B * a.NL, st));
    case M_BL:
      return small ? launch_mode<M_BL, 2, 8>(a, a.B * a.NL * (a.NL - 1), st)
                   : (big ? launch_mode<M_BL, 8, 8>(a, a.B * a.NL * (a.NL - 1), st)
                          : launch_mode<M_BL, 4, 8>(a, a.B * a.NL * (a.NL - 1), st));
  }
  return DD_ERR_BAD_ARG;
}

template <int NW, int MAXT, int KT>
static int launch_node_nw(const AttnArgs& ne, const AttnArgs& nb, const AttnArgs& bl, hipStream_t st) {
  using namespace v2;
  const int N = ne.NP + ne.NL;
  const int n_ne = ne.B * ne_blocks_per_sample(ne.NP, ne.NL, NW), n_nb = (ne.B * ne.NL + NW - 1) / NW;
  int n_bl = (ne.B * ne.NL * (ne.NL - 1) + NW - 1) / NW;
  const int persist = (g_attn_persist && bl.work_counter != nullptr) ? 1 : 0;
  const int32_t* const wf = g_node_trace ? reinterpret_cast<const int32_t*>(g_node_trace) : ne.wait_flags;
  const int wfn = g_node_trace ? -12345 : ne.wait_n;
  AttnArgs blt = bl;
  blt.trip_full = 1 << 27; blt.trip_q = 0;
  auto set_trips = [&](int n_wg) {
    if (ne.nl_real != nullptr || n_wg <= 0) return;
    const int nseg = ne.B * ne.NL * (ne.NL - 1);
    const int full = nseg / (NW * n_wg) * n_wg, rem = nseg - full * NW;
    blt.trip_full = full;
    blt.trip_q = (rem + n_wg - 1) / n_wg;
  };
  if (persist) {
    static int n_cu = 0;
    if (n_cu == 0) {
      int dev = 0;
      hipDeviceProp_t prop;
      if (hipGetDevice(&dev) != hipSuccess || hipGetDeviceProperties(&prop, dev) != hipSuccess) return DD_ERR_HIP;
      n_cu = prop.multiProcessorCount > 0 ? prop.multiProcessorCount : 256;
    }
    if (n_bl > n_cu) n_bl = n_cu;
    if (g_bl_first > 0 && n_bl == n_cu) {
      int want = g_bl_first > 1 ? g_bl_first : (g_node_split_trial >= 0 ? g_node_split_trial : node_split_lookup(ne.B, ne.NP, ne.NL, ne.K));
#if DD_NODE_TRACE
      { static const int env_bl = [] { const char* e = getenv("DD_BL_FIRST"); return e ? atoi(e) : 0; }(); if (env_bl > 0 && g_node_split_trial < 0) want = env_bl; }
#endif
      if (want > 0) {
        n_bl = want < 16 ? 16 : (want > n_cu - 16 ? n_cu - 16 : want);
        set_trips(n_bl);
        if (ne.nl_real != nullptr)
          hipLaunchKernelGGL((k_attn2_node<MAXT, NW, true, KT>), dim3(n_ne + n_nb + n_bl), dim3(NW * 64), 0, st, ne, nb, blt, n_ne, n_nb,
                             persist, n_bl, wf, ne.wait_idx, wfn, 0);
        else
          hipLaunchKernelGGL((k_attn2_node<MAXT, NW, false, KT>), dim3(n_ne + n_nb + n_bl), dim3(NW * 64), 0, st, ne, nb, blt, n_ne, n_nb, persist,
                             n_bl, wf, ne.wait_idx, wfn, 0);
        DD_CHECK_LAUNCH();
        return DD_OK;
      }
    }
  }
  if (persist) set_trips(n_bl);
  if (ne.nl_real != nullptr)
    hipLaunchKernelGGL((k_attn2_node<MAXT, NW, true, KT>), dim3(n_ne + n_nb + n_bl), dim3(NW * 64), 0, st, ne, nb, blt, n_ne, n_nb, persist, 0, wf, ne.wait_idx, wfn, 0);
  else
    hipLaunchKernelGGL((k_attn2_node<MAXT, NW, false, KT>), dim3(n_ne + n_nb + n_bl), dim3(NW * 64), 0, st, ne, nb, blt, n_ne, n_nb, persist, 0, wf, ne.wait_idx, wfn, 0);
  DD_CHECK_LAUNCH();
  return DD_OK;
}
template <int KT>
static int launch_node_kt(const AttnArgs& ne, const AttnArgs& nb, const AttnArgs& bl, hipStream_t st) {
  if (ne.NL > 65) return launch_node_nw<8, 8, KT>(ne, nb, bl, st);
  if (ne.NL > 49) return launch_node_nw<8, 4, KT>(ne, nb, bl, st);
  if (ne.NL > 33) return launch_node_nw<8, 3, KT>(ne, nb, bl, st);
  return launch_node_nw<8, 2, KT>(ne, nb, bl, st);
}
int launch_attn2_node(const AttnArgs& ne, const AttnArgs& nb, const AttnArgs& bl, hipStream_t st) {
  if (ne.NL > 129 || ne.K > DD_KNN_MAX) return DD_ERR_UNSUPPORTED_SHAPE;
  return ne.K <= 32 ? launch_node_kt<2>(ne, nb, bl, st) : launch_node_kt<4>(ne, nb, bl, st);
}
template <int NW, int KT>
static int launch_pos_nw(const AttnArgs& pe, const AttnArgs& pb, hipStream_t st) {
  using namespace v2;
  const int n = (pe.B * pe.NL + NW - 1) / NW;
  if (pe.NL > 65) {
    if constexpr (NW <= 4) {
      if (pe.nl_real != nullptr) hipLaunchKernelGGL((k_attn2_pos<8, NW, true, KT>), dim3(2 * n), dim3(NW * 128), 0, st, pe, pb, n);
      else hipLaunchKernelGGL((k_attn2_pos<8, NW, false, KT>), dim3(2 * n), dim3(NW * 128), 0, st, pe, pb, n);
      DD_CHECK_LAUNCH();
      return DD_OK;
    } else {
      return DD_ERR_UNSUPPORTED_SHAPE;
    }
  }
  if (pe.nl_real != nullptr) {
    if (pe.NL > 49) hipLaunchKernelGGL((k_attn2_pos<4, NW, true, KT>), dim3(2 * n), dim3(NW * 128), 0, st, pe, pb, n);
    else if (pe.NL > 33) hipLaunchKernelGGL((k_attn2_pos<3, NW, true, KT>), dim3(2 * n), dim3(NW * 128), 0, st, pe, pb, n);
    else hipLaunchKernelGGL((k_attn2_pos<2, NW, true, KT>), dim3(2 * n), dim3(NW * 128), 0, st, pe, pb, n);
  } else if (pe.NL > 49) hipLaunchKernelGGL((k_attn2_pos<4, NW, false, KT>), dim3(2 * n), dim3(NW * 128), 0, st, pe, pb, n);
  else if (pe.NL > 33) hipLaunchKernelGGL((k_attn2_pos<3, NW, false, KT>), dim3(2 * n), dim3(NW * 128), 0, st, pe, pb, n);
  else hipLaunchKernelGGL((k_attn2_pos<2, NW, false, KT>), dim3(2 * n), dim3(NW * 128), 0, st, pe, pb, n);
  DD_CHECK_LAUNCH();
  return DD_OK;
}
int g_pos_g_mode = 0;
int launch_attn2_pos_g(const AttnArgs& pe_in, const AttnArgs& pb_in, const GemmArgs* jobs, int njobs, int n_lead, int32_t* counter,
                       hipStream_t st) {
#if !(defined(DD_DEBUG_OPTIONS) && DD_DEBUG_OPTIONS)
  (void)pe_in; (void)pb_in; (void)jobs; (void)njobs; (void)n_lead; (void)counter; (void)st;
  return DD_ERR_UNSUPPORTED_SHAPE;
#else
  using namespace v2;
  if (njobs <= 0 || njobs > 4 || n_lead <= 0 || n_lead > njobs || counter == nullptr) return DD_ERR_BAD_ARG;
  if (pe_in.NL > 65 || pe_in.K > 32 || pe_in.work_counter != nullptr) return DD_ERR_UNSUPPORTED_SHAPE;
  for (int i = 0; i < njobs; ++i)
    if (jobs[i].ln != nullptr || (jobs[i].ldy & 3) || (jobs[i].ncols & 3) || (reinterpret_cast<size_t>(jobs[i].Y) & 15))
      return DD_ERR_UNSUPPORTED_SHAPE;
  PosGemm pg;
  pg.njobs = njobs;
  pg.mode = g_pos_g_mode & 1;
  int total = 0, tiles0 = 0;
  for (int i = 0; i < 4; ++i) {
    const GemmArgs& g = jobs[i < njobs ? i : 0];
    pg.job[i] = g;
    pg.nbx[i] = i < njobs ? (g.rows + GT - 1) / GT : 1;
    if (i < njobs) total += pg.nbx[i] * ((g.ncols + GT - 1) / GT);
    pg.end[i] = total;
    if (i + 1 == n_lead) tiles0 = total;
  }
  constexpr int NW = 4;
  const int n = (pe_in.B * pe_in.NL + NW - 1) / NW, n_att = 2 * n;
  const int n_g0 = (tiles0 + 1) / 2, n_g1 = (total - tiles0 + 1) / 2;
  AttnArgs pe = pe_in, pb = pb_in;
  pe.wait_flags = pb.wait_flags = counter; pe.wait_idx = pb.wait_idx = 0; pe.wait_n = pb.wait_n = (g_pos_g_mode & 2) ? -tiles0 : tiles0;
  const dim3 grid(n_g0 + n_att + n_g1), block(NW * 128);
  if (pe.nl_real != nullptr) {
    if (pe.NL > 49) hipLaunchKernelGGL((k_attn2_pos_g<4, NW, true>), grid, block, 0, st, pe, pb, n, pg, n_g0, tiles0, n_att, total, counter);
    else if (pe.NL > 33) hipLaunchKernelGGL((k_attn2_pos_g<3, NW, true>), grid, block, 0, st, pe, pb, n, pg, n_g0, tiles0, n_att, total, counter);
    else hipLaunchKernelGGL((k_attn2_pos_g<2, NW, true>), grid, block, 0, st, pe, pb, n, pg, n_g0, tiles0, n_att, total, counter);
  } else if (pe.NL > 49) hipLaunchKernelGGL((k_attn2_pos_g<4, NW>), grid, block, 0, st, pe, pb, n, pg, n_g0, tiles0, n_att, total, counter);
  else if (pe.NL > 33) hipLaunchKernelGGL((k_attn2_pos_g<3, NW>), grid, block, 0, st, pe, pb, n, pg, n_g0, tiles0, n_att, total, counter);
  else hipLaunchKernelGGL((k_attn2_pos_g<2, NW>), grid, block, 0, st, pe, pb, n, pg, n_g0, tiles0, n_att, total, counter);
  DD_CHECK_LAUNCH();
  return DD_OK;
#endif
}

int g_pos_waves = 4;
int launch_attn2_pos(const AttnArgs& pe, const AttnArgs& pb, hipStream_t st) {
  if (pe.NL > 129 || pe.K > DD_KNN_MAX) return DD_ERR_UNSUPPORTED_SHAPE;
  if (pe.K > 32) return launch_pos_nw<4, 4>(pe, pb, st);
  if (pe.NL > 65 && g_pos_waves > 4) return launch_pos_nw<4, 2>(pe, pb, st);
  if (g_pos_waves == 2) return launch_pos_nw<2, 2>(pe, pb, st);
  if (g_pos_waves == 4) return launch_pos_nw<4, 2>(pe, pb, st);
  return launch_pos_nw<8, 2>(pe, pb, st);
}

}
#endif
```

### decompdiff_amd/csrc/dd_graph.hip

```cpp
#include "dd_kernels.hpp"

namespace dd {


__device__ __forceinline__ bool atom_is_real(int n, int NP, int npb, int nlb) { return n < NP ? n < npb : (n - NP) < nlb; }

struct PosView {
  const float* p;
  const float* l;
  int NP;
  __device__ __forceinline__ float get(int n, int c) const { return n < NP ? p[3 * n + c] : l[3 * (n - NP) + c]; }
};

template <int CAND>
__device__ __forceinline__ void knn_wave(const PosView& pv, int i, int N, int K, int32_t* __restrict__ nbr_row, bool masked, int npb,
                                         int nlb, unsigned long long* sel , int32_t* srt ) {
  const int lane = threadIdx.x & 63;
  const float cx = pv.get(i, 0), cy = pv.get(i, 1), cz = pv.get(i, 2);
  unsigned khi[CAND], klo[CAND];
#pragma unroll
  for (int t = 0; t < CAND; ++t) {
    const int c = lane + 64 * t;
    khi[t] = ~0u; klo[t] = ~0u;
    if (c < N && c != i && (!masked || atom_is_real(c, pv.NP, npb, nlb))) {
// ... 517 lines not shown
  int n = B * NL * 3;
  hipLaunchKernelGGL(k_xupdate, dim3((n + 255) / 256), dim3(256), 0, st, x, dxe, dxb, B, NP, NL, x_next);
  DD_CHECK_LAUNCH();
  return DD_OK;
}

int launch_knn(const float* x, int B, int N, int K, int32_t* nbr, hipStream_t st, int NP, const int32_t* np_real,
               const int32_t* nl_real) {
  const dim3 grid((B * N + 3) / 4), block(256);
  const int cand = (N + 63) / 64;
  if (NP < 0) { NP = N; np_real = nl_real = nullptr; }
  if (cand <= 2) hipLaunchKernelGGL(k_knn<2>, grid, block, 0, st, x, B, N, K, nbr, NP, np_real, nl_real);
  else if (cand <= 4) hipLaunchKernelGGL(k_knn<4>, grid, block, 0, st, x, B, N, K, nbr, NP, np_real, nl_real);
  else if (cand <= 6) hipLaunchKernelGGL(k_knn<6>, grid, block, 0, st, x, B, N, K, nbr, NP, np_real, nl_real);
  else if (cand <= 11) hipLaunchKernelGGL(k_knn<11>, grid, block, 0, st, x, B, N, K, nbr, NP, np_real, nl_real);
  else if (cand <= 16) hipLaunchKernelGGL(k_knn<16>, grid, block, 0, st, x, B, N, K, nbr, NP, np_real, nl_real);
  else hipLaunchKernelGGL(k_knn<DD_N_MAX / 64>, grid, block, 0, st, x, B, N, K, nbr, NP, np_real, nl_real);
  DD_CHECK_LAUNCH();
  return DD_OK;
}
int launch_edge_weights(const float* x, const int32_t* nbr, int B, int N, int K, const float* W1T, const float* b1,
                        const float* ln, const float* w2, const float* b2, float* ew, hipStream_t st, int NP, const int32_t* np_real,
                        const int32_t* nl_real) {
  if (NP < 0) { NP = N; np_real = nl_real = nullptr; }
  hipLaunchKernelGGL(k_edge_weights2, dim3((B * N + 3) / 4), dim3(256), 0, st, x, nbr, B, N, K, W1T, b1, ln, w2, b2, ew, NP, np_real, nl_real);
  DD_CHECK_LAUNCH();
  return DD_OK;
}
int launch_embed_all(const float* protein_h, const float* protein_pos, const float* lig_pos, const int32_t* lig_v,
                     const float* lig_aux, const float* Wl, const float* bl, int B, int NP, int NL, float* h, float* xa, float* xb,
                     const int32_t* bond, long bond_rows, const float* Wb, const float* bb, float* hb, int32_t* counters,
                     hipStream_t st, int32_t* advance, int nv) {
  const long nn = (long)B * (NP + NL) * 128, nb = bond_rows * 128;
  const int node_blocks = (int)((nn + 255) / 256), bond_blocks = (int)((nb + 255) / 256);
  hipLaunchKernelGGL(k_embed_all, dim3(node_blocks + bond_blocks), dim3(256), 0, st, protein_h, protein_pos, lig_pos, lig_v, lig_aux,
                     Wl, bl, B, NP, NL, h, xa, xb, bond, bond_rows, Wb, bb, hb, counters, node_blocks, advance, nv);
  DD_CHECK_LAUNCH();
  return DD_OK;
}
template <int KW>
static void launch_head_graph(const HeadArgs& a, int N, dim3 grid, dim3 block, hipStream_t st) {
  const int cand = (N + 63) / 64;
  if (cand <= 2) hipLaunchKernelGGL((k_head_graph<2, KW>), grid, block, 0, st, a);
  else if (cand <= 4) hipLaunchKernelGGL((k_head_graph<4, KW>), grid, block, 0, st, a);
  else if (cand <= 6) hipLaunchKernelGGL((k_head_graph<6, KW>), grid, block, 0, st, a);
  else if (cand <= 11) hipLaunchKernelGGL((k_head_graph<11, KW>), grid, block, 0, st, a);
  else if (cand <= 16) hipLaunchKernelGGL((k_head_graph<16, KW>), grid, block, 0, st, a);
  else hipLaunchKernelGGL((k_head_graph<DD_N_MAX / 64, KW>), grid, block, 0, st, a);
}
int launch_head_all(const float* protein_h, const float* protein_pos, const float* lig_pos, const int32_t* lig_v,
                    const float* lig_aux, const float* Wl, const float* bl, int B, int NP, int NL, int K, float* h, float* xa, float* xb,
                    const int32_t* bond, long bond_rows, const float* Wb, const float* bb, float* hb, int32_t* counters,
                    int32_t* advance, int32_t* nbr, float* ew, const float* EW_W1T, const float* EW_b1, const float* EW_ln,
                    const float* EW_w2, const float* EW_b2, const int32_t* np_real, const int32_t* nl_real, const float* l0_tables,
                    float* l0_P, float* PL, float* l0_qn, float* qlnb, float* PB, float* qb, hipStream_t st, int parts, int nv) {
  if (K > DD_KNN_MAX || (parts & 3) == 0 || (l0_tables != nullptr && nv != DD_NUM_V)) return DD_ERR_UNSUPPORTED_SHAPE;
  const int N = NP + NL;
  HeadArgs a;
  a.B = B; a.NP = NP; a.NL = NL; a.K = K;
  a.protein_pos = protein_pos; a.lig_pos = lig_pos; a.nbr = nbr; a.ew = ew;
  a.EW_W1T = EW_W1T; a.EW_b1 = EW_b1; a.EW_ln = EW_ln; a.EW_w2 = EW_w2; a.EW_b2 = EW_b2;
  a.np_real = np_real; a.nl_real = nl_real;
  a.protein_h = protein_h; a.lig_v = lig_v; a.lig_aux = lig_aux; a.Wl = Wl; a.bl = bl; a.h = h; a.xa = xa; a.xb = xb;
  a.bond = bond; a.bond_rows = bond_rows; a.Wb = Wb; a.bb = bb; a.hb = hb; a.counters = counters; a.advance = advance;
  a.nv = nv;
  a.tab = l0_tables; a.l0_P = l0_P; a.PL = PL; a.l0_qn = l0_qn; a.qlnb = qlnb; a.PB = PB; a.qb = qb;
  const long nn = (long)B * N * 128, nb = bond_rows * 128;
  a.n_embed_nodes = (int)((nn + 255) / 256);
  a.n_embed = a.n_embed_nodes + (int)((nb + 255) / 256);
  a.n_graph = (B * N + 3) / 4;
  a.atom_f4 = (long)B * NL * (160 + 320 + 32 + 32);
  const long bond_f4 = (long)B * NL * (NL - 1) * (160 + 32);
  const int n_l0 = l0_tables ? (int)((a.atom_f4 + bond_f4 + 255) / 256) : 0;
  const dim3 block(256);
  if (parts & 2) hipLaunchKernelGGL(k_head_rows, dim3((unsigned)(a.n_embed + n_l0)), block, 0, st, a);
  if (parts & 1) {
    const dim3 grid((unsigned)a.n_graph);
    if (K <= 32) launch_head_graph<32>(a, N, grid, block, st);
    else launch_head_graph<64>(a, N, grid, block, st);
  }
  DD_CHECK_LAUNCH();
  return DD_OK;
}
int launch_layer0_rows(const float* tables, const int32_t* lig_v, const float* lig_aux, const int32_t* bond, int B, int NP, int NL,
                       float* l0_P, float* PL, float* l0_qn, float* qlnb, float* PB, float* qb, hipStream_t st) {
  const long atom_f4 = (long)B * NL * (160 + 320 + 32 + 32), bond_f4 = (long)B * NL * (NL - 1) * (160 + 32);
  hipLaunchKernelGGL(k_layer0_rows, dim3((unsigned)((atom_f4 + bond_f4 + 255) / 256)), dim3(256), 0, st, tables, lig_v, lig_aux, bond,
                     B, NP, NL, l0_P, PL, l0_qn, qlnb, PB, qb, atom_f4);
  DD_CHECK_LAUNCH();
  return DD_OK;
}
int launch_bl_assemble(const float* x, const float* PB, const float* PL, const float* Wgp, int B, int NP, int NL, float* Ek, float* Ev,
                       float* q1, float* Rk, float* Rv, hipStream_t st, const float* xprev, const float* dxe, const float* dxb,
                       float* xout, FlagWait fw) {
  if (Wgp == nullptr) return DD_ERR_BAD_ARG;
  const long rows = (long)B * NL * (NL - 1);
  const long tiles = (rows + 15) / 16;
  const int bpo = (int)((tiles + 3) / 4);
  hipLaunchKernelGGL(k_bl_assemble3, dim3((unsigned)(bpo * (q1 ? 5 : 4))), dim3(256), 0, st, x, PB, PL, Wgp, B, NP, NL, Ek, Ev, q1,
                     Rk, Rv, bpo, xprev, dxe, dxb, xout, fw);
  DD_CHECK_LAUNCH();
  return DD_OK;
}

}

extern "C" int dd_knn(const float* x, int B, int N, int K, int32_t* nbr, void* stream) {
  if (!x || !nbr || B <= 0 || N <= 1) return DD_ERR_BAD_ARG;
  if (N > DD_N_MAX || K > DD_KNN_MAX || K > N - 1 || K <= 0) return DD_ERR_UNSUPPORTED_SHAPE;
  return dd::launch_knn(x, B, N, K, nbr, (hipStream_t)stream);
}

extern "C" int dd_knn_masked(const float* x, int B, int NP, int NL, int K, const int32_t* np_real, const int32_t* nl_real, int32_t* nbr,
                             void* stream) {
  const int N = NP + NL;
  if (!x || !nbr || !nl_real || B <= 0 || NP < 0 || NL <= 0 || K <= 0 || K > DD_KNN_MAX || K > N - 1 || N > DD_N_MAX) return DD_ERR_BAD_ARG;
  return dd::launch_knn(x, B, N, K, nbr, (hipStream_t)stream, NP, np_real, nl_real);
}

extern "C" int dd_knn_csr(const float* x, const int32_t* ptr, int B, int n, int n_max, int K, int loop, const int64_t* out_off,
                          int64_t E, int64_t* edge_index, void* stream) {
  if (!ptr || !out_off || B <= 0 || n < 0 || E < 0 || K <= 0 || (loop != 0 && loop != 1)) return DD_ERR_BAD_ARG;
  if (K > DD_KNN_MAX) return DD_ERR_UNSUPPORTED_SHAPE;
  if (n == 0 || E == 0) return DD_OK;
  if (!x || !edge_index) return DD_ERR_BAD_ARG;
  const dim3 grid((unsigned)(((long)n + 3) / 4)), block(256);
  hipStream_t st = (hipStream_t)stream;
  const int cand = (n_max + 63) / 64;
#define DD_KNN_CSR(C) hipLaunchKernelGGL(dd::k_knn_csr<C>, grid, block, 0, st, x, ptr, B, n, K, loop, out_off, (long)E, edge_index)
  if (cand <= 2) DD_KNN_CSR(2);
  else if (cand <= 4) DD_KNN_CSR(4);
  else if (cand <= 8) DD_KNN_CSR(8);
  else if (cand <= 16) DD_KNN_CSR(16);
  else DD_KNN_CSR(DD_N_MAX / 64);
#undef DD_KNN_CSR
  DD_CHECK_LAUNCH();
  return DD_OK;
}

extern "C" int dd_edge_weights(const float* x, const int32_t* nbr, int B, int N, int K, const float* W1T,
                               const float* b1, const float* ln, const float* w2, const float* b2, float* ew,
                               void* stream) {
  if (!x || !nbr || !W1T || !b1 || !ln || !w2 || !b2 || !ew) return DD_ERR_BAD_ARG;
  return dd::launch_edge_weights(x, nbr, B, N, K, W1T, b1, ln, w2, b2, ew, (hipStream_t)stream);
}

extern "C" int dd_embed_protein(const float* protein_v, int rows, const float* W, const float* b, float* protein_h,
                                void* stream) {
  if (!protein_v || !W || !b || !protein_h || rows <= 0) return DD_ERR_BAD_ARG;
  long n = (long)rows * 128;
  hipLaunchKernelGGL(dd::k_embed_protein, dim3((unsigned)((n + 255) / 256)), dim3(256), 0, (hipStream_t)stream,
                     protein_v, rows, W, b, protein_h);
  DD_CHECK_LAUNCH();
  return DD_OK;
}
```

### decompdiff_amd/csrc/dd_kernels.hpp

```cpp
#pragma once
#include "dd_common.hpp"

namespace dd {

struct FlagWait { const int32_t* flags; int idx0, n0, idx1, n1; };
inline FlagWait no_wait() { return FlagWait{nullptr, -1, 0, -1, 0}; }

struct GemmArgs {
  const float* X; int x_rows_per_b; long x_stride_b; int ldx; int rows;
  const float* W; const float* bias; const float* ln;
  float* Y; int y_rows_per_b; long y_stride_b; int ldy; int ncols; int accumulate;
  const float* X2; int x2_N, x2_NP;
  int x2_Eb, x2_NLm1, x2_ld;
  long long* dbg;
  const float* acc_src;
};
inline GemmArgs gemm_args(const float* X, int x_rows_per_b, long x_stride_b, int ldx, int rows, const float* W,
                          const float* bias, const float* ln, float* Y, int y_rows_per_b, long y_stride_b, int ldy,
                          int ncols, int accumulate) {
  GemmArgs g{X, x_rows_per_b, x_stride_b, ldx, rows, W, bias, ln, Y, y_rows_per_b, y_stride_b, ldy, ncols, accumulate,
             nullptr, 0, 0, 0, 0, 0, nullptr, nullptr};
  return g;
}
enum { DD_FLAG_TICKET = 0, DD_FLAG_LIN = 1, DD_FLAG_TICKET2 = 2, DD_FLAG_PL1 = 3, DD_FLAG_P1Q = 4, DD_FLAG_PBQ = 5, DD_FLAG_PB1R = 6,
       DD_FLAG_NODE = 7, DD_FLAGS_PER_LAYER = 8 };
constexpr int DD_FLAG_LAYERS = 8;
constexpr int DD_FLAG_STRIDE = 32;
constexpr int DD_FLAG_ERR = DD_FLAG_LAYERS * DD_FLAGS_PER_LAYER * DD_FLAG_STRIDE;
#if defined(DD_DEBUG_OPTIONS) && DD_DEBUG_OPTIONS
constexpr int DD_NUM_FLAGS = DD_FLAG_ERR + DD_FLAG_STRIDE;
#else
constexpr int DD_NUM_FLAGS = 0;
#endif
constexpr int DD_NUM_COUNTERS = 192;
constexpr int DD_TAIL_CHUNK = 2;
constexpr int DD_TAIL_MAX_JOBS = 14;
struct TailJob {
  GemmArgs g;
  int nbx, tiles;
  int wait0, wait0_n, wait1, wait1_n;
  int sig;
};
struct TailArgs {
  TailJob job[DD_TAIL_MAX_JOBS];
  int end[DD_TAIL_MAX_JOBS];
  int njobs, total, ticket, persist;
  int32_t* flags;
};
inline TailJob tail_job(const GemmArgs& g, int wait0 = -1, int wait0_n = 0, int sig = -1, int wait1 = -1, int wait1_n = 0) {
  TailJob q{g, 0, 0, wait0, wait0_n, wait1, wait1_n, sig};
  return q;
}
inline int gemm_tiles(int rows, int cols) { return ((rows + 63) / 64) * ((cols + 63) / 64); }
int launch_gemm_tail(TailArgs& ta, hipStream_t st);
int launch_gemm128(const GemmArgs& a, hipStream_t st);
int launch_gemm128_batch(const GemmArgs* jobs, int njobs, hipStream_t st);
struct NodeOutArgs { const float* Ae; const float* Ab; const float* h; float* out; const float* blk; int B, NP, NL; };
int launch_node_out_fc(const NodeOutArgs& a, hipStream_t st);

int launch_embed_all(const float* protein_h, const float* protein_pos, const float* lig_pos, const int32_t* lig_v,
                     const float* lig_aux, const float* Wl, const float* bl, int B, int NP, int NL, float* h, float* xa, float* xb,
                     const int32_t* bond, long bond_rows, const float* Wb, const float* bb, float* hb, int32_t* counters,
                     hipStream_t st, int32_t* advance = nullptr, int nv = DD_NUM_V);
int launch_drift_armsca(const float* lig_pos, const int32_t* decomp_index, int B, int NL, float min_d, float max_d,
                        float* grad, int accumulate, int norm_B, hipStream_t st);
int launch_drift_arms_repul(const float* lig_pos, const int32_t* decomp_index, int B, int NL, float max_d, int mode, float* grad,
                            int accumulate, int norm_B, hipStream_t st);
int launch_drift_clash(const float* lig_pos, const float* offset, const float* full_protein_pos, int B, int NL, int NF,
                       float sigma, float gamma, float* grad, int accumulate, const int32_t* nl_real, hipStream_t st);
int launch_knn(const float* x, int B, int N, int K, int32_t* nbr, hipStream_t st, int NP = -1, const int32_t* np_real = nullptr,
               const int32_t* nl_real = nullptr);
int launch_edge_weights(const float* x, const int32_t* nbr, int B, int N, int K, const float* W1T, const float* b1,
                        const float* ln, const float* w2, const float* b2, float* ew, hipStream_t st, int NP = -1,
                        const int32_t* np_real = nullptr, const int32_t* nl_real = nullptr);
int launch_bl_assemble(const float* x, const float* PB, const float* PL, const float* Wgp, int B, int NP, int NL, float* Ek, float* Ev,
                       float* q1, float* Rk, float* Rv, hipStream_t st, const float* xprev = nullptr, const float* dxe = nullptr,
                       const float* dxb = nullptr, float* xout = nullptr, FlagWait fw = FlagWait{nullptr, -1, 0, -1, 0});
int launch_layer0_rows(const float* tables, const int32_t* lig_v, const float* lig_aux, const int32_t* bond, int B, int NP, int NL,
                       float* l0_P, float* PL, float* l0_qn, float* qlnb, float* PB, float* qb, hipStream_t st);
int launch_head_all(const float* protein_h, const float* protein_pos, const float* lig_pos, const int32_t* lig_v,
                    const float* lig_aux, const float* Wl, const float* bl, int B, int NP, int NL, int K, float* h, float* xa, float* xb,
                    const int32_t* bond, long bond_rows, const float* Wb, const float* bb, float* hb, int32_t* counters,
                    int32_t* advance, int32_t* nbr, float* ew, const float* EW_W1T, const float* EW_b1, const float* EW_ln,
                    const float* EW_w2, const float* EW_b2, const int32_t* np_real, const int32_t* nl_real, const float* l0_tables,
                    float* l0_P, float* PL, float* l0_qn, float* qlnb, float* PB, float* qb, hipStream_t st, int parts = 3,
                    int nv = DD_NUM_V);
int launch_extract_ligand(const float* x, int B, int NP, int NL, float* out, hipStream_t st);

enum { M_NE = 0, M_NB = 1, M_BL = 2, M_PE = 3, M_PB = 4 };

struct AttnArgs {
  int B, NP, NL, K;
  const float* x;
  const int32_t* nbr;
  const float* ew;
  const float *kd, *ks, *vd, *vs, *ke, *ve;
  int ld_kd, ld_ks, ld_vd, ld_vs, ld_ke, ld_ve;
  const float* q;
  const float *Akp, *Avp;
  const float *Wakp, *Wavp;
  const float *lnk, *lnv;
  const float* W2k;
  const float* b2v;
  const float* W2v;
  const float *qhid, *lnq, *W2q, *b2q; int ld_qhid;
  int* work_counter;
  const float *W2v16, *b2v16;
  float* out;
  const float* dxe;
  float* x_next;
  const float *Rk, *Rv;
  long long* dbg_clock;
  int out_assign;
  const int32_t *np_real, *nl_real, *bl_prefix;
  const int32_t* wait_flags; int wait_idx, wait_n;
  int trip_full, trip_q;
  const float *lin_W, *lin_b, *lin_add;
};

int launch_attn2(int mode, const AttnArgs& a, hipStream_t st);
int launch_attn2_node(const AttnArgs& ne, const AttnArgs& nb, const AttnArgs& bl, hipStream_t st);
int launch_attn2_pos(const AttnArgs& pe, const AttnArgs& pb, hipStream_t st);
int launch_attn2_pos_g(const AttnArgs& pe, const AttnArgs& pb, const GemmArgs* jobs, int njobs, int n_lead, int32_t* counter,
                       hipStream_t st);
int launch_xupdate(const float* x, const float* dxe, const float* dxb, int B, int NP, int NL, float* x_next, hipStream_t st);

struct StepRowsArgs {
  const float* hid;
  const float* logits_in;
  const float* W2;
  const float* b2;
  int rows, NC, rows_per_sample;
  const float* tab;
  int T;
  const int32_t* step_counter;
  int counter_bias;
  int32_t* state;
  const float* uniforms;
  uint32_t stream_id;
  float* logits_out;
  float* traj_recon;
  float* traj_prob;
  int32_t* traj_state;
};
struct StepPosArgs {
  int B, NL, T;
  const int32_t* step_counter;
  int counter_bias;
  const float* x0;
  const float* x0_prev; const float* x0_dxe; const float* x0_dxb; float* x0_out; int NP;
  float* xt;
  const float* tab_pos;
  const float* tab_score;
  const float* atom_std;
  const float* offset;
  const float* grad_a; int scale_a;
  const float* grad_c; int scale_c;
  const float* grad_r; int scale_r;
  const float* eps;
  float* traj_pos;
};
int launch_step_rows(const StepRowsArgs& a, hipStream_t st);
int launch_step_pos(const StepPosArgs& a, hipStream_t st);
int launch_advance(int32_t* ctr, hipStream_t st);
int launch_reset_run_state(int32_t* rs, int t_start, uint64_t seed, hipStream_t st);
int launch_step_all(const StepRowsArgs& rb, const StepRowsArgs& rv, const StepPosArgs& p, hipStream_t st);

}
```

### decompdiff_amd/hip_lib.py

```python
from __future__ import annotations

import ctypes
import os
from ctypes import POINTER, c_char_p, c_float, c_int, c_int32, c_int64, c_long, c_size_t, c_uint64, c_void_p

import torch

_HERE = os.path.dirname(os.path.abspath(__file__))
LIB_PATH = os.environ.get("DD_HIP_LIB") or os.path.join(_HERE, "lib", "libdecompdiff_hip.so")

EXPORTED_SYMBOLS = [
    "dd_status_string", "dd_abi_version", "dd_weights_form", "dd_build_flags", "dd_workspace_floats", "dd_knn", "dd_knn_masked", "dd_knn_csr", "dd_edge_weights", "dd_gemm128",
    "dd_gemm128_tn", "dd_gemm128_tn_bias", "dd_gemm128_tn_scratch_floats",
    "dd_ln_relu_scratch_floats", "dd_ln_relu_forward", "dd_ln_relu_backward",
    "dd_embed_protein", "dd_forward", "dd_sample_steps", "dd_sample_steps_graph", "dd_sample_steps_graph_multi",
    "dd_graph_create", "dd_graph_launch", "dd_graph_destroy",
    "dd_drift_armsca", "dd_drift_clash", "dd_drift_arms_repul",
    "dd_attn_aggregate_node", "dd_attn_aggregate_triplet", "dd_attn_aggregate_pos", "dd_reverse_step",
    "dd_segment_reduce", "dd_segment_softmax", "dd_sampler_reset",
    "dd_layer0_tables", "dd_layer0_prepare",
    "dd_forward_ex", "dd_sample_steps_ex", "dd_sample_steps_graph_ex", "dd_graph_create_ex", "dd_sample_steps_graph_multi_ex",
    "dd_node_out_fc",
    "dd_forward_ex2", "dd_sample_steps_ex2", "dd_sample_steps_graph_ex2", "dd_graph_create_ex2", "dd_sample_steps_graph_multi_ex2",
]
DEBUG_SYMBOLS = [
    "dd_workspace_view", "dd_profile_step", "dd_debug_set_clock_buffer", "dd_debug_set_fusion", "dd_debug_set_option",
    "dd_debug_node_split", "dd_debug_node_split_cache_path", "dd_debug_schedule", "dd_debug_philox", "dd_debug_options_epoch", "dd_queue_error",
]
MEASUREMENT_ONLY_SYMBOLS = ("dd_queue_error",)
BUILD_DEBUG_OPTIONS, BUILD_EXACT_MATH = 1, 2


class DDSampler(ctypes.Structure):
    _fields_ = [
        ("B", c_int32), ("NP", c_int32), ("NL", c_int32), ("K", c_int32), ("NF", c_int32),
        ("num_layers", c_int32), ("T", c_int32), ("t_start", c_int32),
        ("weights", c_void_p), ("slot_off", c_void_p),
        ("tab_pos", c_void_p), ("tab_v", c_void_p), ("tab_b", c_void_p), ("tab_score", c_void_p),
        ("protein_pos", c_void_p), ("protein_h", c_void_p), ("lig_aux", c_void_p), ("atom_std", c_void_p),
        ("offset", c_void_p), ("decomp_index", c_void_p), ("full_protein_pos", c_void_p),
        ("lig_pos", c_void_p), ("lig_v", c_void_p), ("lig_bond", c_void_p), ("step_counter", c_void_p),
        ("drift_armsca", c_int32), ("armsca_min_d", c_float), ("armsca_max_d", c_float), ("armsca_scale", c_int32),
        ("drift_clash", c_int32), ("clash_sigma", c_float), ("clash_gamma", c_float), ("clash_scale", c_int32),
        ("drift_norm_batch", c_int32),
        ("u_v", c_void_p), ("u_b", c_void_p), ("eps", c_void_p), ("seed", c_uint64),
        ("traj_pos", c_void_p), ("traj_v", c_void_p), ("traj_bond", c_void_p), ("traj_v0", c_void_p),
        ("traj_vt", c_void_p), ("traj_bt", c_void_p),
        ("pred_pos", c_void_p), ("pred_v", c_void_p), ("pred_bond", c_void_p),
        ("workspace", c_void_p), ("workspace_floats", c_size_t),
        ("np_real", c_void_p), ("nl_real", c_void_p), ("bl_prefix", c_void_p),
        ("l0_tables", c_void_p), ("l0_P", c_void_p), ("l0_qn", c_void_p),
        ("num_v", c_int32), ("drift_repul", c_int32), ("repul_max_d", c_float), ("repul_scale", c_int32),
    ]


BOND_HEAD_LIN, BOND_HEAD_PRE_ATT = 0, 1


class DDBondHead(ctypes.Structure):
    _fields_ = [("kind", c_int32), ("num_r", c_int32), ("W_p", c_void_p), ("W_r", c_void_p), ("b1", c_void_p),
                ("offset", c_void_p), ("coeff", c_float), ("reserved", c_int32)]


class DDNodeOut(ctypes.Structure):
    _fields_ = [("num_layers", c_int32), ("reserved", c_int32), ("layer", c_void_p * 64)]


L0_TABLE_FLOATS = 16 * 640 + 16 * 1280 + 5 * 640 + 16 * 128 + 16 * 128 + 80 * 128


class DDWsView(ctypes.Structure):
    _fields_ = [("x", c_void_p), ("h", c_void_p), ("hb", c_void_p), ("ew", c_void_p), ("A", c_void_p),
                ("nbr", c_void_p), ("Anb", c_void_p), ("lin_in_node", ctypes.c_int32)]


PROF_CATS = ["misc", "gemm", "assemble", "attn_NE", "attn_NB", "attn_BL", "attn_PE", "attn_PB", "step", "event_pair"]


ABI_VERSION = 9


class HipLibraryError(RuntimeError):
    pass


_lib = None


def load():
    global _lib
    if _lib is not None:
        return _lib
    if not os.path.exists(LIB_PATH):
        raise HipLibraryError(f"{LIB_PATH} not found: build it with `python -m decompdiff_amd.build`; "
                              "there is no CPU fallback for the sampling hot path")
    try:
        lib = ctypes.CDLL(LIB_PATH)
    except OSError as e:
        raise HipLibraryError(f"could not load {LIB_PATH}: {e}") from e
    lib.dd_status_string.restype = c_char_p
    lib.dd_status_string.argtypes = [c_int]
    lib.dd_abi_version.restype = c_int
    ignore_abi = os.environ.get("DD_IGNORE_ABI") == "1"
    if lib.dd_abi_version() != ABI_VERSION and not ignore_abi:
        raise HipLibraryError(f"{LIB_PATH} has ABI version {lib.dd_abi_version()}, this package needs {ABI_VERSION}: rebuild it")
    S = POINTER(DDSampler)
    protos = {
        "dd_build_flags": [],
        "dd_weights_form": [],
        "dd_workspace_floats": [c_int, c_int, c_int, c_int],
        "dd_knn": [c_void_p, c_int, c_int, c_int, c_void_p, c_void_p],
        "dd_knn_masked": [c_void_p, c_int, c_int, c_int, c_int, c_void_p, c_void_p, c_void_p, c_void_p],
        "dd_knn_csr": [c_void_p, c_void_p, c_int, c_int, c_int, c_int, c_int, c_void_p, c_int64, c_void_p, c_void_p],
        "dd_edge_weights": [c_void_p, c_void_p, c_int, c_int, c_int] + [c_void_p] * 7,
        "dd_gemm128": [c_void_p, c_int, c_long, c_int, c_int, c_void_p, c_void_p, c_void_p, c_void_p, c_int, c_long, c_int, c_int,
                       c_int, c_void_p],
        "dd_gemm128_tn_scratch_floats": [c_long, c_int],
        "dd_gemm128_tn": [c_void_p, c_int, c_int, c_void_p, c_int, c_long, c_void_p, c_void_p, c_int, c_int, c_void_p],
        "dd_gemm128_tn_bias": [c_void_p, c_int, c_int, c_void_p, c_int, c_long, c_void_p, c_void_p, c_int, c_int, c_void_p, c_void_p],
        "dd_ln_relu_scratch_floats": [c_long],
        "dd_ln_relu_forward": [c_void_p, c_void_p, c_void_p, c_void_p, c_void_p, c_long, c_void_p],
        "dd_ln_relu_backward": [c_void_p] * 9 + [c_long, c_void_p],
        "dd_embed_protein": [c_void_p, c_int, c_void_p, c_void_p, c_void_p, c_void_p],
        "dd_forward": [S, c_void_p],
        "dd_sampler_reset": [S, c_void_p],
        "dd_layer0_tables": [S, c_void_p, c_void_p],
        "dd_layer0_prepare": [S, c_void_p],
        "dd_debug_options_epoch": [],
        "dd_queue_error": [S, c_void_p, POINTER(c_int)],
        "dd_sample_steps": [S, c_int, c_void_p],
        "dd_sample_steps_graph": [S, c_int, c_void_p],
        "dd_graph_create": [S, c_int, c_void_p, POINTER(c_void_p)],
        "dd_graph_launch": [c_void_p, c_int, c_void_p],
        "dd_graph_destroy": [c_void_p],
        "dd_sample_steps_graph_multi": [POINTER(S), c_int, c_int, POINTER(c_void_p)],
        "dd_forward_ex": [S, POINTER(DDBondHead), c_void_p],
        "dd_sample_steps_ex": [S, POINTER(DDBondHead), c_int, c_void_p],
        "dd_sample_steps_graph_ex": [S, POINTER(DDBondHead), c_int, c_void_p],
        "dd_graph_create_ex": [S, POINTER(DDBondHead), c_int, c_void_p, POINTER(c_void_p)],
        "dd_sample_steps_graph_multi_ex": [POINTER(S), POINTER(POINTER(DDBondHead)), c_int, c_int, POINTER(c_void_p)],
        "dd_node_out_fc": [c_void_p, c_void_p, c_void_p, c_int, c_int, c_int, c_void_p, c_void_p, c_void_p, c_void_p, c_void_p],
        "dd_forward_ex2": [S, POINTER(DDBondHead), POINTER(DDNodeOut), c_void_p],
        "dd_sample_steps_ex2": [S, POINTER(DDBondHead), POINTER(DDNodeOut), c_int, c_void_p],
        "dd_sample_steps_graph_ex2": [S, POINTER(DDBondHead), POINTER(DDNodeOut), c_int, c_void_p],
        "dd_graph_create_ex2": [S, POINTER(DDBondHead), POINTER(DDNodeOut), c_int, c_void_p, POINTER(c_void_p)],
        "dd_sample_steps_graph_multi_ex2": [POINTER(S), POINTER(POINTER(DDBondHead)), POINTER(POINTER(DDNodeOut)), c_int, c_int,
                                            POINTER(c_void_p)],
        "dd_drift_armsca": [c_void_p, c_void_p, c_int, c_int, c_float, c_float, c_void_p, c_int, c_void_p],
        "dd_drift_clash": [c_void_p, c_void_p, c_void_p, c_int, c_int, c_int, c_float, c_float, c_void_p, c_int, c_void_p],
        "dd_drift_arms_repul": [c_void_p, c_void_p, c_int, c_int, c_float, c_int, c_void_p, c_int, c_void_p],
        "dd_workspace_view": [S, POINTER(DDWsView)],
        "dd_debug_set_clock_buffer": [c_void_p, c_int],
        "dd_debug_set_fusion": [c_int],
        "dd_debug_set_option": [c_int, c_int],
        "dd_debug_node_split": [c_int, c_int, c_int, c_int],
        "dd_debug_node_split_cache_path": [c_char_p, c_int],
        "dd_debug_schedule": [],
        "dd_reverse_step": [S, c_void_p, c_void_p, c_void_p, c_void_p],
        "dd_attn_aggregate_node": [c_void_p, c_int, c_void_p, c_void_p, c_void_p, c_void_p, c_int, c_void_p, c_void_p],
        "dd_attn_aggregate_triplet": [c_void_p, c_void_p, c_void_p, c_void_p, c_int, c_void_p, c_void_p],
        "dd_attn_aggregate_pos": [c_void_p, c_void_p, c_void_p, c_void_p, c_void_p, c_void_p, c_int, c_void_p, c_void_p],
        "dd_segment_reduce": [c_void_p, c_void_p, c_int, c_int, c_int, c_long, c_void_p, c_void_p, c_void_p],
        "dd_segment_softmax": [c_void_p, c_void_p, c_int, c_int, c_void_p, c_void_p],
        "dd_debug_philox": [c_uint64, c_int, c_long, c_int, c_void_p, c_void_p],
        "dd_profile_step": [S, c_int, POINTER(c_float), c_void_p],
    }
    restypes = {"dd_workspace_floats": c_size_t, "dd_gemm128_tn_scratch_floats": c_size_t, "dd_ln_relu_scratch_floats": c_size_t}
    for name in EXPORTED_SYMBOLS + DEBUG_SYMBOLS:
        if name in ("dd_status_string", "dd_abi_version"):
            continue
        if not hasattr(lib, name):
            if ignore_abi or name in MEASUREMENT_ONLY_SYMBOLS:
                continue
            raise HipLibraryError(f"{LIB_PATH} does not export {name}: rebuild it")
        fn = getattr(lib, name)
        if name in protos:
            fn.argtypes = protos[name]
        fn.restype = restypes.get(name, c_int)
    _lib = lib
    return lib


def check(rc: int, what: str = ""):
    if rc != 0:
        msg = load().dd_status_string(rc).decode()
        raise RuntimeError(f"decompdiff_hip {what} failed: {msg} (status {rc})")


def ptr(t):
    if t is None:
        return None
    assert t.is_contiguous(), "decompdiff_hip needs contiguous tensors"
    return ctypes.c_void_p(t.data_ptr())


def stream_ptr(device=None):
    return ctypes.c_void_p(torch.cuda.current_stream(device).cuda_stream)


def require_gpu(t: torch.Tensor, name: str):
    if not t.is_cuda:
        raise HipLibraryError(f"{name} must live on a HIP device (got {t.device}); the sampling hot path has no "
                              "CPU implementation in this package")


def weights_form() -> int:
    lib = load()
    return int(lib.dd_weights_form()) if hasattr(lib, "dd_weights_form") else 0


def is_measurement_build() -> bool:
    lib = load()
    if not hasattr(lib, "dd_build_flags"):
        return False
    return bool(lib.dd_build_flags() & BUILD_DEBUG_OPTIONS)
```

### include/decompdiff_hip_debug.h

```cpp
#ifndef DECOMPDIFF_HIP_DEBUG_H
#define DECOMPDIFF_HIP_DEBUG_H

#include "decompdiff_hip.h"

#ifdef __cplusplus
extern "C" {
#endif

typedef enum dd_prof_cat {
  DD_PROF_MISC, DD_PROF_GEMM, DD_PROF_ASSEMBLE, DD_PROF_ATTN_NE, DD_PROF_ATTN_NB, DD_PROF_ATTN_BL, DD_PROF_ATTN_PE,
  DD_PROF_ATTN_PB, DD_PROF_STEP,
  DD_PROF_EVENT_PAIR,
  DD_NUM_PROF_CATS
} dd_prof_cat;
int dd_profile_step(const dd_sampler* s, int n_iters, float* ms_per_category , void* stream);

int dd_debug_set_clock_buffer(long long* buf, int mode);
int dd_debug_set_fusion(int mode);
int dd_debug_set_option(int key, int value);
int dd_debug_options_epoch(void);
int dd_debug_node_split(int B, int NP, int NL, int K);
int dd_debug_node_split_cache_path(char* out, int cap);
int dd_debug_schedule(void);
#if defined(DD_DEBUG_OPTIONS) && DD_DEBUG_OPTIONS
int dd_queue_error(const dd_sampler* s, void* stream, int* code);
#endif

int dd_debug_philox(uint64_t seed, int step, long rows, int kind, float* out, void* stream);

typedef struct dd_ws_view {
  float *x, *h, *hb, *ew, *A;
  int32_t* nbr;
  float* Anb;
  int32_t lin_in_node;
} dd_ws_view;
int dd_workspace_view(const dd_sampler* s, dd_ws_view* out);

#ifdef __cplusplus
}
#endif
#endif
```

Measured before the change: 885.6.

## Prune protein node-edge attention rows in last layer to ligand-referenced nodes

Adds a kernel that builds, per sample, a compact list of protein nodes that appear in ligand atoms' kNN neighbourhoods. The final layer's node-edge attention then processes only those live protein rows, since only ligand outputs are consumed downstream. It also autotunes a separate block split for the pruned kernel and caches it by kind. This adds a small extra kernel on the side stream, plus extra autotune time and a new cache format.

```diff
diff --git a/decompdiff_amd/csrc/dd_api.hip b/decompdiff_amd/csrc/dd_api.hip
--- a/decompdiff_amd/csrc/dd_api.hip
+++ b/decompdiff_amd/csrc/dd_api.hip
@@ -16,6 +16,7 @@
   float *xa, *xb, *h, *hb, *ew, *P, *PL, *PB, *P2, *PL2, *PB2, *Ek, *Ev, *Rk, *Rv, *q1bl, *qn, *ql, *ql2, *qlnb, *qb, *A, *Anb, *dxe, *dxb, *ga, *gc, *gr, *h2, *hs;
   int32_t* nbr;
   int32_t* counters;
+  int32_t *live, *live_count;
   size_t total;
 };
 
@@ -62,6 +63,8 @@
   w.h2 = w.hs = nullptr;
 #endif
   w.counters = reinterpret_cast<int32_t*>(take(DD_NUM_COUNTERS + DD_NUM_FLAGS));
+  w.live = reinterpret_cast<int32_t*>(take(B * (size_t)NP + B));
+  w.live_count = w.live ? w.live + B * (size_t)NP : nullptr;
   w.total = off;
   return w;
 }
@@ -156,6 +159,8 @@
 DD_OPT g_side_lin = DD_SIDE_LIN_DEFAULT;
 static int g_lin_in_node = [] { const char* e = getenv("DD_LIN_IN_NODE"); return e ? (e[0] == '1' ? 1 : (e[0] == '0' ? 0 : -1)) : -1; }();
 static int g_lin_proj_main = [] { const char* e = getenv("DD_LIN_PROJ_MAIN"); return e ? (e[0] == '1' ? 1 : 0) : 0; }();
+static int g_prune_last = 1;
+static int g_prune_force = 0;
 static bool lin_in_node_for(int B, int NL) {
   if (g_lin_in_node >= 0) return g_lin_in_node != 0;
   return (long)B * NL * (NL - 1) < 8L * 256 * 2;
@@ -530,6 +535,7 @@
   const bool l0 = fused && g_l0_tables && g_q1_in_gemm && g_gemm_ksplit_on() && s->l0_tables && s->l0_P && s->l0_qn &&
                   s->nl_real == nullptr;
   int32_t* advance = (fold && fold->advance) ? s->step_counter : nullptr;
+  const bool prune = (fold != nullptr || g_prune_force) && g_prune_last && fused && NP > 0 && attn2_node_prunes(NL);
   bool head_join = false;
   if (overlap && g_head_fused) {
     auto head = [&](hipStream_t sx, int parts) -> int {
@@ -542,6 +548,7 @@
     if (hipEventRecord(g_ev_fork[8], st) != hipSuccess || hipStreamWaitEvent(g_side, g_ev_fork[8], 0) != hipSuccess) return DD_ERR_HIP;
     if (g_head_rows_first) DD_TRYP(DD_PROF_MISC, head(st, 2));
     DD_TRYP(DD_PROF_MISC, head(g_side, 1));
+    if (prune) DD_TRYP(DD_PROF_MISC, launch_live_rows(w.nbr, B, NP, NL, K, s->np_real, s->nl_real, w.live, w.live_count, g_side));
     if (hipEventRecord(g_ev_join[8], g_side) != hipSuccess) return DD_ERR_HIP;
     head_join = true;
     if (!g_head_rows_first) DD_TRYP(DD_PROF_MISC, head(st, 2));
@@ -560,6 +567,7 @@
     DD_TRYP(DD_PROF_MISC, launch_knn(w.xa, B, N, K, w.nbr, gs, NP, s->np_real, s->nl_real));
     DD_TRYP(DD_PROF_MISC, launch_edge_weights(w.xa, w.nbr, B, N, K, GW(DD_G_EW_W1T), GW(DD_G_EW_b1), GW(DD_G_EW_ln), GW(DD_G_EW_w2),
                                GW(DD_G_EW_b2), w.ew, gs, NP, s->np_real, s->nl_real));
+    if (prune) DD_TRYP(DD_PROF_MISC, launch_live_rows(w.nbr, B, NP, NL, K, s->np_real, s->nl_real, w.live, w.live_count, gs));
     if (overlap) {
       if (hipEventRecord(g_ev_join[8], g_side) != hipSuccess) return DD_ERR_HIP;
       head_join = true;
@@ -677,7 +685,8 @@
       bl.W2k = LW(l, DD_BL_W2k); bl.W2v = LW(l, DD_BL_W2v); bl.b2v = LW(l, DD_BL_b2v); bl.out = w.hb;
       bl.Rk = w.Rk; bl.Rv = w.Rv;
       bl.work_counter = (l < 64) ? w.counters + l : nullptr;
-      DD_TRYP(DD_PROF_ATTN_BL, launch_attn2_node(ne, nb, bl, st));
+      const bool live = prune && l + 1 == s->num_layers;
+      DD_TRYP(DD_PROF_ATTN_BL, launch_attn2_node(ne, nb, bl, st, live ? w.live : nullptr, live ? w.live_count : nullptr));
     }
     if (ahead_split && l + 1 < s->num_layers && hipEventRecord(g_ev_qa_fork[l + 1], st) != hipSuccess) return DD_ERR_HIP;
     const bool side_lin = g_side_lin && ahead_split && ahead_b2 && l + 1 < s->num_layers;
@@ -1134,6 +1143,7 @@
   out->x = (s->num_layers & 1) ? w.xb : w.xa;
   out->h = w.h; out->hb = w.hb; out->ew = w.ew; out->A = w.A; out->nbr = w.nbr;
   out->Anb = (dd::g_fuse && s->NL <= dd::g_fused_max_nl) ? w.Anb : nullptr;
+  out->live = w.live; out->live_count = w.live_count;
   out->lin_in_node = 0;
   if (out->Anb && dd::lin_in_node_for(s->B, s->NL) && dd::g_lin_with_pb2 && !dd::g_side_lin && dd::g_heads_early) {
     out->lin_in_node = 1;
@@ -1169,9 +1179,9 @@
 }
 
 namespace dd {
-extern int g_node_split_trial;
-int node_split_lookup(int B, int NP, int NL, int K);
-void node_split_store(int B, int NP, int NL, int K, int n_bl);
+extern int g_node_split_trial, g_node_split_trial_kind;
+int node_split_lookup(int B, int NP, int NL, int K, int kind);
+void node_split_store(int B, int NP, int NL, int K, int kind, int n_bl);
 bool node_split_applies(int B, int NL, int n_cu);
 }
 
@@ -1194,17 +1204,23 @@
   snprintf(tag, sizeof(tag), "_cu%d_abi%d_%08x", n_cu, dd_abi_version(), h);
   return dir + "/node_split_" + name + tag + ".txt";
 }
-static int node_split_cache_read(const std::string& path, int B, int NP, int NL, int K) {
+static int node_split_cache_read(const std::string& path, int B, int NP, int NL, int K, int kind) {
   if (path.empty()) return -1;
   FILE* f = fopen(path.c_str(), "r");
   if (!f) return -1;
-  int b, np, nl, k, n, found = -1;
-  while (fscanf(f, "%d %d %d %d %d", &b, &np, &nl, &k, &n) == 5)
-    if (b == B && np == NP && nl == NL && k == K) found = n;
+  int found = -1;
+  char buf[256];
+  while (fgets(buf, sizeof(buf), f)) {
+    int v[6], extra;
+    const int n = sscanf(buf, "%d %d %d %d %d %d %d", &v[0], &v[1], &v[2], &v[3], &v[4], &v[5], &extra);
+    if (n != 5 && n != 6) continue;
+    const int kd = n == 6 ? v[4] : 0, n_bl = n == 6 ? v[5] : v[4];
+    if (v[0] == B && v[1] == NP && v[2] == NL && v[3] == K && kd == kind) found = n_bl;
+  }
   fclose(f);
   return found;
 }
-static void node_split_cache_append(const std::string& path, int B, int NP, int NL, int K, int n_bl) {
+static void node_split_cache_append(const std::string& path, int B, int NP, int NL, int K, int kind, int n_bl) {
   if (path.empty()) return;
   const size_t slash = path.rfind('/');
   if (slash != std::string::npos) {
@@ -1219,7 +1235,8 @@
     fclose(f);
   }
   char line[96];
-  snprintf(line, sizeof(line), "%d %d %d %d %d\n", B, NP, NL, K, n_bl);
+  if (kind == 0) snprintf(line, sizeof(line), "%d %d %d %d %d\n", B, NP, NL, K, n_bl);
+  else snprintf(line, sizeof(line), "%d %d %d %d %d %d\n", B, NP, NL, K, kind, n_bl);
   all += line;
   char tmp[32];
   snprintf(tmp, sizeof(tmp), ".tmp%d", (int)getpid());
@@ -1231,6 +1248,7 @@
   if (!ok || rename(t.c_str(), path.c_str()) != 0) (void)unlink(t.c_str());
 }
 
+static int autotune_node_split_pruned(const dd_sampler* s, hipStream_t st, int n_cu, const std::string& cache_path);
 static int autotune_node_split(const dd_sampler* s, hipStream_t st) {
   static int n_cu = 0;
   if (n_cu == 0) {
@@ -1242,13 +1260,14 @@
   const bool fused = dd::g_fuse && s->NL <= dd::g_fused_max_nl && dd::g_dbg_clock == nullptr;
   static const bool enabled = [] { const char* e = getenv("DD_NODE_SPLIT_AUTOTUNE"); return !(e && e[0] == '0'); }();
   if (!enabled) return DD_OK;
-  if (!fused || !dd::node_split_applies(s->B, s->NL, n_cu) || dd::node_split_lookup(s->B, s->NP, s->NL, s->K) >= 0) return DD_OK;
+  if (!fused || !dd::node_split_applies(s->B, s->NL, n_cu)) return DD_OK;
   const std::string cache_path = node_split_cache_path(n_cu);
+  if (dd::node_split_lookup(s->B, s->NP, s->NL, s->K, 0) >= 0) return autotune_node_split_pruned(s, st, n_cu, cache_path);
   {
-    const int cached = node_split_cache_read(cache_path, s->B, s->NP, s->NL, s->K);
+    const int cached = node_split_cache_read(cache_path, s->B, s->NP, s->NL, s->K, 0);
     if (cached == 0 || (cached >= 16 && cached <= n_cu - 16 && cached % 8 == 0)) {
-      dd::node_split_store(s->B, s->NP, s->NL, s->K, cached);
-      return DD_OK;
+      dd::node_split_store(s->B, s->NP, s->NL, s->K, 0, cached);
+      return autotune_node_split_pruned(s, st, n_cu, cache_path);
     }
   }
   hipEvent_t e0, e1;
@@ -1256,6 +1275,7 @@
   int rc = DD_OK;
   auto time_split = [&](int n_bl, float& best) {
     dd::g_node_split_trial = n_bl;
+    dd::g_node_split_trial_kind = 0;
     best = 1e30f;
     for (int rep = 0; rep < 3 && rc == DD_OK; ++rep) {
       if (hipEventRecord(e0, st) != hipSuccess) { rc = DD_ERR_HIP; break; }
@@ -1312,8 +1332,61 @@
   (void)hipEventDestroy(e0);
   (void)hipEventDestroy(e1);
   if (rc == DD_OK) {
-    dd::node_split_store(s->B, s->NP, s->NL, s->K, best_n);
-    node_split_cache_append(cache_path, s->B, s->NP, s->NL, s->K, best_n);
+    dd::node_split_store(s->B, s->NP, s->NL, s->K, 0, best_n);
+    node_split_cache_append(cache_path, s->B, s->NP, s->NL, s->K, 0, best_n);
+    rc = autotune_node_split_pruned(s, st, n_cu, cache_path);
+  }
+  return rc;
+}
+
+static int autotune_node_split_pruned(const dd_sampler* s, hipStream_t st, int n_cu, const std::string& cache_path) {
+  if (!dd::g_prune_last || s->NP <= 0 || !dd::attn2_node_prunes(s->NL) || dd::node_split_lookup(s->B, s->NP, s->NL, s->K, 1) >= 0) return DD_OK;
+  const int full = dd::node_split_lookup(s->B, s->NP, s->NL, s->K, 0);
+  if (full <= 0) return DD_OK;
+  {
+    const int cached = node_split_cache_read(cache_path, s->B, s->NP, s->NL, s->K, 1);
+    if (cached >= 16 && cached <= n_cu - 16 && cached % 8 == 0) {
+      dd::node_split_store(s->B, s->NP, s->NL, s->K, 1, cached);
+      return DD_OK;
+    }
+  }
+  hipEvent_t e0, e1;
+  if (hipEventCreate(&e0) != hipSuccess || hipEventCreate(&e1) != hipSuccess) return DD_ERR_HIP;
+  int rc = DD_OK;
+  dd::g_prune_force = 1;
+  auto time_split = [&](int n_bl, float& best) {
+    dd::g_node_split_trial = n_bl;
+    dd::g_node_split_trial_kind = 1;
+    best = 1e30f;
+    for (int rep = 0; rep < 3 && rc == DD_OK; ++rep) {
+      if (hipEventRecord(e0, st) != hipSuccess) { rc = DD_ERR_HIP; break; }
+      rc = dd::forward_impl(s, st);
+      if (rc != DD_OK) break;
+      float ms = 0.f;
+      if (hipEventRecord(e1, st) != hipSuccess || hipEventSynchronize(e1) != hipSuccess ||
+          hipEventElapsedTime(&ms, e0, e1) != hipSuccess) { rc = DD_ERR_HIP; break; }
+      if (rep > 0 && ms < best) best = ms;
+    }
+  };
+  int best_n = full;
+  float best_t = 1e30f, t = 0.f;
+  for (int n = full; n <= n_cu - 16 && n <= full + 64 && rc == DD_OK; n += 16) {
+    time_split(n, t);
+    if (t < best_t) { best_t = t; best_n = n; }
+  }
+  for (int n : {best_n - 8, best_n + 8}) {
+    if (rc != DD_OK || n < 16 || n > n_cu - 16) continue;
+    time_split(n, t);
+    if (t < best_t) { best_t = t; best_n = n; }
+  }
+  dd::g_node_split_trial = -1;
+  dd::g_node_split_trial_kind = 0;
+  dd::g_prune_force = 0;
+  (void)hipEventDestroy(e0);
+  (void)hipEventDestroy(e1);
+  if (rc == DD_OK) {
+    dd::node_split_store(s->B, s->NP, s->NL, s->K, 1, best_n);
+    node_split_cache_append(cache_path, s->B, s->NP, s->NL, s->K, 1, best_n);
   }
   return rc;
 }
@@ -1612,13 +1685,17 @@
 }
 #endif
 
-extern "C" int dd_debug_node_split(int B, int NP, int NL, int K) { return dd::node_split_lookup(B, NP, NL, K); }
+extern "C" int dd_debug_node_split(int B, int NP, int NL, int K) { return dd::node_split_lookup(B, NP, NL, K, 0); }
+extern "C" int dd_debug_node_split_kind(int B, int NP, int NL, int K, int kind) {
+  return (kind == 0 || kind == 1) ? dd::node_split_lookup(B, NP, NL, K, kind) : -1;
+}
 
 extern "C" int dd_debug_schedule(void) { return dd::g_p2_in_pos ? 1 : 0; }
 
 extern "C" int dd_debug_set_option(int key, int value) {
   ++g_options_epoch;
   if (key == 0) return dd_debug_set_fusion(value);
+  if (key == 34) { dd::g_prune_last = value ? 1 : 0; return DD_OK; }
 #if defined(DD_DEBUG_OPTIONS) && DD_DEBUG_OPTIONS
   if (key == 1) { dd::g_gemm_ksplit = value ? 1 : 0; return DD_OK; }
   if (key == 3) { dd::g_attn_persist = value ? 1 : 0; return DD_OK; }
diff --git a/decompdiff_amd/csrc/dd_attention2.hip b/decompdiff_amd/csrc/dd_attention2.hip
--- a/decompdiff_amd/csrc/dd_attention2.hip
+++ b/decompdiff_amd/csrc/dd_attention2.hip
@@ -260,13 +260,15 @@
 __host__ __device__ inline int ne_blocks_per_sample(int NP, int NL, int NW) { return (NP + NW - 1) / NW + (NL + NW - 1) / NW; }
 
 template <int MODE, int MAXT, int NW, bool PERSIST = false, bool RAG = false, bool PAIR = false, bool STAMPS = true, bool WIDE = false,
-          typename ARGS = AttnArgs>
-__device__ __forceinline__ void attn2_body(const ARGS& a, const int block, float* smem) {
+          bool LIVE = false, typename ARGS = AttnArgs>
+__device__ __forceinline__ void attn2_body(const ARGS& a, const int block, float* smem, const int32_t* live = nullptr,
+                                           const int32_t* live_count = nullptr) {
   constexpr bool KNN = (MODE == M_NE || MODE == M_PE);
   constexpr bool POS = (MODE == M_PE || MODE == M_PB);
   constexpr bool TRIP = (MODE == M_BL);
   constexpr bool BOND = (MODE == M_NB || MODE == M_PB);
   static_assert(!PAIR || (POS && !PERSIST), "wave pairs: coordinate modes");
+  static_assert(!LIVE || (MODE == M_NE && !PERSIST), "live-row list: node_layer_with_edge blocks");
   constexpr int NT = (PAIR ? 2 : 1) * NW * 64;
   using L = Lds<MODE>;
   constexpr int LNP = L::LNP, WAO = L::WAO;
@@ -297,6 +299,16 @@
     const int first = wg_protein ? ne_rb * NW : (ne_rb - ne_nbp) * NW;
     if (first >= (wg_protein ? (a.np_real ? a.np_real[ne_b] : a.NP) : a.nl_real[ne_b])) return;
   }
+  int live_n = 0;
+  if (LIVE && wg_protein && ne_b < a.B) {
+    live_n = live_count[ne_b];
+    if (ne_rb * NW >= live_n) return;
+  }
+  auto live_node = [&](int i) -> int {
+    if (!wg_protein) return a.NP + (ne_rb - ne_nbp) * NW + i;
+    const int k = ne_rb * NW + i;
+    return k < live_n ? live[(long)ne_b * a.NP + k] : a.NP;
+  };
   long long* dbg = (STAMPS && a.dbg_clock) ? a.dbg_clock + (long)block * 16 : nullptr;
 #define DD_STAMP(i) do { if (dbg && threadIdx.x == 0) dbg[i] = (long long)__builtin_amdgcn_s_memtime(); } while (0)
   DD_STAMP(0);
@@ -359,7 +371,7 @@
     }
     seg = wave < cnt ? bl_dense_seg(base + wave) : a.B * Eb;
   } else if (MODE == M_NE) {
-    const int nd = wg_protein ? ne_rb * NW + wave : a.NP + (ne_rb - ne_nbp) * NW + wave;
+    const int nd = LIVE ? live_node(wave) : (wg_protein ? ne_rb * NW + wave : a.NP + (ne_rb - ne_nbp) * NW + wave);
     seg = (nd < (wg_protein ? a.NP : N) && ne_b < a.B) ? ne_b * N + nd : nseg;
   } else {
     seg = block * NW + wave;
@@ -870,7 +882,7 @@
       for (int r = 0; r < 4; ++r) {
         const int i = 4 * cg + r;
         if (MODE == M_NE) {
-          const int nd = wg_protein ? ne_rb * NW + i : a.NP + (ne_rb - ne_nbp) * NW + i;
+          const int nd = LIVE ? live_node(i) : (wg_protein ? ne_rb * NW + i : a.NP + (ne_rb - ne_nbp) * NW + i);
           bool ok = nd < (wg_protein ? a.NP : N) && ne_b < a.B;
           if (RAG && ok) ok = nd < a.NP ? nd < (a.np_real ? a.np_real[ne_b] : a.NP) : nd - a.NP < a.nl_real[ne_b];
           if (ok) {
@@ -926,7 +938,7 @@
 #pragma unroll
     for (int u = 0; u < 2; ++u) {
       const int sI = 2 * cg + u;
-      const int nd = wg_protein ? ne_rb * NW + sI : a.NP + (ne_rb - ne_nbp) * NW + sI;
+      const int nd = LIVE ? live_node(sI) : (wg_protein ? ne_rb * NW + sI : a.NP + (ne_rb - ne_nbp) * NW + sI);
       bool ok = nd < (wg_protein ? a.NP : N) && ne_b < a.B;
       if (RAG && ok) ok = nd < a.NP ? nd < (a.np_real ? a.np_real[ne_b] : a.NP) : nd - a.NP < a.nl_real[ne_b];
       const float val = fmaf(bias2, SS[sI * 16 + 2 * wave + eh], eh ? d[2 * u + 1] : d[2 * u]);
@@ -1013,9 +1025,10 @@
 
 constexpr int imax(int a, int b) { return a > b ? a : b; }
 
-template <int MAXT, int NW, bool RAG = false, int KT = 2>
+template <int MAXT, int NW, bool RAG = false, int KT = 2, bool LIVE = false>
 __global__ __launch_bounds__(NW * 64) void k_attn2_node(const AttnArgs ne, const AttnArgs nb, const AttnArgs bl, int n_ne, int n_nb,
-                                                        int persist, int n_bl_first, const int32_t* wflags, int widx, int wn, int nep) {
+                                                        int persist, int n_bl_first, const int32_t* wflags, int widx, int wn, int nep,
+                                                        const int32_t* live, const int32_t* live_count) {
   constexpr int SZ = imax(imax(Lds<M_NE>::TOTAL, Lds<M_NB>::TOTAL), Lds<M_BL>::TOTAL) + 12;
   __shared__ __attribute__((aligned(16))) float smem[SZ];
   int blk = blockIdx.x;
@@ -1049,11 +1062,11 @@
       return;
     }
     blk -= n_bl_first;
-    if (blk < n_ne) { attn2_body<M_NE, KT, NW, false, RAG, false, false, (KT > 2)>(args(0), blk, smem); DD_TRACE_END(0); }
+    if (blk < n_ne) { attn2_body<M_NE, KT, NW, false, RAG, false, false, (KT > 2), LIVE>(args(0), blk, smem, live, live_count); DD_TRACE_END(0); }
     else { attn2_body<M_NB, MAXT, NW, false, RAG, false, false, (KT > 2)>(args(1), blk - n_ne, smem); DD_TRACE_END(1); }
     return;
   }
-  if (blk < n_ne) attn2_body<M_NE, KT, NW, false, RAG, false, false, (KT > 2)>(args(0), blk, smem);
+  if (blk < n_ne) attn2_body<M_NE, KT, NW, false, RAG, false, false, (KT > 2), LIVE>(args(0), blk, smem, live, live_count);
   else if (blk < n_ne + n_nb) attn2_body<M_NB, MAXT, NW, false, RAG, false, false, (KT > 2)>(args(1), blk - n_ne, smem);
   else if (persist) attn2_body<M_BL, MAXT, NW, true, RAG, false, false, (KT > 2)>(args(2), blk - n_ne - n_nb, smem);
   else attn2_body<M_BL, MAXT, NW, false, RAG, false, false, (KT > 2)>(args(2), blk - n_ne - n_nb, smem);
@@ -1139,7 +1152,8 @@
 #endif
 
 #ifdef DD_ASM_ONLY
-template __global__ void k_attn2_node<2, 8, false>(const AttnArgs, const AttnArgs, const AttnArgs, int, int, int, int, const int32_t*, int, int, int);
+template __global__ void k_attn2_node<2, 8, false>(const AttnArgs, const AttnArgs, const AttnArgs, int, int, int, int, const int32_t*, int, int, int, const int32_t*, const int32_t*);
+template __global__ void k_attn2_node<2, 8, false, 2, true>(const AttnArgs, const AttnArgs, const AttnArgs, int, int, int, int, const int32_t*, int, int, int, const int32_t*, const int32_t*);
 template __global__ void k_attn2_pos<2, 4, false>(const AttnArgs, const AttnArgs, int);
 }
 }
@@ -1164,20 +1178,22 @@
 int g_bl_first = 1;
 int g_node_split_trial = -1;
 long long* g_node_trace = nullptr;
+int g_node_split_trial_kind = 0;
 namespace {
-struct NodeSplit { int B, NP, NL, K, n_bl; };
+struct NodeSplit { int B, NP, NL, K, kind, n_bl; };
 std::vector<NodeSplit> g_node_splits;
 }
-int node_split_lookup(int B, int NP, int NL, int K) {
+int node_split_lookup(int B, int NP, int NL, int K, int kind) {
   for (const NodeSplit& e : g_node_splits)
-    if (e.B == B && e.NP == NP && e.NL == NL && e.K == K) return e.n_bl;
+    if (e.B == B && e.NP == NP && e.NL == NL && e.K == K && e.kind == kind) return e.n_bl;
   return -1;
 }
-void node_split_store(int B, int NP, int NL, int K, int n_bl) {
+void node_split_store(int B, int NP, int NL, int K, int kind, int n_bl) {
   for (NodeSplit& e : g_node_splits)
-    if (e.B == B && e.NP == NP && e.NL == NL && e.K == K) { e.n_bl = n_bl; return; }
-  g_node_splits.push_back(NodeSplit{B, NP, NL, K, n_bl});
-}
+    if (e.B == B && e.NP == NP && e.NL == NL && e.K == K && e.kind == kind) { e.n_bl = n_bl; return; }
+  g_node_splits.push_back(NodeSplit{B, NP, NL, K, kind, n_bl});
+}
+bool attn2_node_prunes(int NL) { return NL <= 33; }
 bool node_split_applies(int B, int NL, int n_cu) {
   return g_attn_persist && g_bl_first == 1 && (B * NL * (NL - 1) + 7) / 8 >= n_cu;
 }
@@ -1207,7 +1223,7 @@
 }
 
 template <int NW, int MAXT, int KT>
-static int launch_node_nw(const AttnArgs& ne, const AttnArgs& nb, const AttnArgs& bl, hipStream_t st) {
+static int launch_node_nw(const AttnArgs& ne, const AttnArgs& nb, const AttnArgs& bl, hipStream_t st, const int32_t* live_rows, const int32_t* live_count) {
   using namespace v2;
   const int N = ne.NP + ne.NL;
   const int n_ne = ne.B * ne_blocks_per_sample(ne.NP, ne.NL, NW), n_nb = (ne.B * ne.NL + NW - 1) / NW;
@@ -1224,6 +1240,27 @@
     blt.trip_full = full;
     blt.trip_q = (rem + n_wg - 1) / n_wg;
   };
+  const bool live = live_rows != nullptr;
+  if (live && (MAXT != 2 || live_count == nullptr)) return DD_ERR_BAD_ARG;
+  auto launch = [&](int n_bl_first) -> int {
+    const dim3 grid(n_ne + n_nb + n_bl), block(NW * 64);
+#define DD_NODE_LAUNCH(RAG, LIVE) \
+    hipLaunchKernelGGL((k_attn2_node<MAXT, NW, RAG, KT, LIVE>), grid, block, 0, st, ne, nb, blt, n_ne, n_nb, persist, n_bl_first, wf, ne.wait_idx, wfn, 0, \
+                       live_rows, live_count)
+    if constexpr (MAXT == 2) {
+      if (live) {
+        if (ne.nl_real != nullptr) DD_NODE_LAUNCH(true, true);
+        else DD_NODE_LAUNCH(false, true);
+        DD_CHECK_LAUNCH();
+        return DD_OK;
+      }
+    }
+    if (ne.nl_real != nullptr) DD_NODE_LAUNCH(true, false);
+    else DD_NODE_LAUNCH(false, false);
+#undef DD_NODE_LAUNCH
+    DD_CHECK_LAUNCH();
+    return DD_OK;
+  };
   if (persist) {
     static int n_cu = 0;
     if (n_cu == 0) {
@@ -1234,42 +1271,32 @@
     }
     if (n_bl > n_cu) n_bl = n_cu;
     if (g_bl_first > 0 && n_bl == n_cu) {
-      int want = g_bl_first > 1 ? g_bl_first : (g_node_split_trial >= 0 ? g_node_split_trial : node_split_lookup(ne.B, ne.NP, ne.NL, ne.K));
+      const int kind = live ? 1 : 0;
+      int want = g_bl_first > 1 ? g_bl_first : ((g_node_split_trial >= 0 && g_node_split_trial_kind == kind) ? g_node_split_trial : node_split_lookup(ne.B, ne.NP, ne.NL, ne.K, kind));
+      if (want < 0 && live) want = node_split_lookup(ne.B, ne.NP, ne.NL, ne.K, 0);
 #if DD_NODE_TRACE
       { static const int env_bl = [] { const char* e = getenv("DD_BL_FIRST"); return e ? atoi(e) : 0; }(); if (env_bl > 0 && g_node_split_trial < 0) want = env_bl; }
 #endif
       if (want > 0) {
         n_bl = want < 16 ? 16 : (want > n_cu - 16 ? n_cu - 16 : want);
         set_trips(n_bl);
-        if (ne.nl_real != nullptr)
-          hipLaunchKernelGGL((k_attn2_node<MAXT, NW, true, KT>), dim3(n_ne + n_nb + n_bl), dim3(NW * 64), 0, st, ne, nb, blt, n_ne, n_nb,
-                             persist, n_bl, wf, ne.wait_idx, wfn, 0);
-        else
-          hipLaunchKernelGGL((k_attn2_node<MAXT, NW, false, KT>), dim3(n_ne + n_nb + n_bl), dim3(NW * 64), 0, st, ne, nb, blt, n_ne, n_nb, persist,
-                             n_bl, wf, ne.wait_idx, wfn, 0);
-        DD_CHECK_LAUNCH();
-        return DD_OK;
+        return launch(n_bl);
       }
     }
   }
   if (persist) set_trips(n_bl);
-  if (ne.nl_real != nullptr)
-    hipLaunchKernelGGL((k_attn2_node<MAXT, NW, true, KT>), dim3(n_ne + n_nb + n_bl), dim3(NW * 64), 0, st, ne, nb, blt, n_ne, n_nb, persist, 0, wf, ne.wait_idx, wfn, 0);
-  else
-    hipLaunchKernelGGL((k_attn2_node<MAXT, NW, false, KT>), dim3(n_ne + n_nb + n_bl), dim3(NW * 64), 0, st, ne, nb, blt, n_ne, n_nb, persist, 0, wf, ne.wait_idx, wfn, 0);
-  DD_CHECK_LAUNCH();
-  return DD_OK;
+  return launch(0);
 }
 template <int KT>
-static int launch_node_kt(const AttnArgs& ne, const AttnArgs& nb, const AttnArgs& bl, hipStream_t st) {
-  if (ne.NL > 65) return launch_node_nw<8, 8, KT>(ne, nb, bl, st);
-  if (ne.NL > 49) return launch_node_nw<8, 4, KT>(ne, nb, bl, st);
-  if (ne.NL > 33) return launch_node_nw<8, 3, KT>(ne, nb, bl, st);
-  return launch_node_nw<8, 2, KT>(ne, nb, bl, st);
-}
-int launch_attn2_node(const AttnArgs& ne, const AttnArgs& nb, const AttnArgs& bl, hipStream_t st) {
+static int launch_node_kt(const AttnArgs& ne, const AttnArgs& nb, const AttnArgs& bl, hipStream_t st, const int32_t* live, const int32_t* live_count) {
+  if (ne.NL > 65) return launch_node_nw<8, 8, KT>(ne, nb, bl, st, live, live_count);
+  if (ne.NL > 49) return launch_node_nw<8, 4, KT>(ne, nb, bl, st, live, live_count);
+  if (ne.NL > 33) return launch_node_nw<8, 3, KT>(ne, nb, bl, st, live, live_count);
+  return launch_node_nw<8, 2, KT>(ne, nb, bl, st, live, live_count);
+}
+int launch_attn2_node(const AttnArgs& ne, const AttnArgs& nb, const AttnArgs& bl, hipStream_t st, const int32_t* live, const int32_t* live_count) {
   if (ne.NL > 129 || ne.K > DD_KNN_MAX) return DD_ERR_UNSUPPORTED_SHAPE;
-  return ne.K <= 32 ? launch_node_kt<2>(ne, nb, bl, st) : launch_node_kt<4>(ne, nb, bl, st);
+  return ne.K <= 32 ? launch_node_kt<2>(ne, nb, bl, st, live, live_count) : launch_node_kt<4>(ne, nb, bl, st, live, live_count);
 }
 template <int NW, int KT>
 static int launch_pos_nw(const AttnArgs& pe, const AttnArgs& pb, hipStream_t st) {
diff --git a/decompdiff_amd/csrc/dd_graph.hip b/decompdiff_amd/csrc/dd_graph.hip
--- a/decompdiff_amd/csrc/dd_graph.hip
+++ b/decompdiff_amd/csrc/dd_graph.hip
@@ -623,6 +623,39 @@
   DD_CHECK_LAUNCH();
   return DD_OK;
 }
+__global__ __launch_bounds__(256) void k_live_rows(const int32_t* __restrict__ nbr, int B, int NP, int NL, int K,
+                                                   const int32_t* __restrict__ np_real, const int32_t* __restrict__ nl_real,
+                                                   int32_t* __restrict__ live, int32_t* __restrict__ count) {
+  __shared__ int flag[DD_N_MAX];
+  const int b = blockIdx.x, N = NP + NL;
+  const int np = np_real ? np_real[b] : NP, nl = nl_real ? nl_real[b] : NL;
+  for (int i = threadIdx.x; i < NP; i += 256) flag[i] = 0;
+  __syncthreads();
+  const int32_t* rows = nbr + ((long)b * N + NP) * K;
+  for (int i = threadIdx.x; i < nl * K; i += 256) {
+    const int j = rows[i];
+    if (j >= 0 && j < np) flag[j] = 1;
+  }
+  __syncthreads();
+  if (threadIdx.x >= 64) return;
+  const int lane = threadIdx.x;
+  int n = 0;
+  for (int base = 0; base < NP; base += 64) {
+    const int r = base + lane;
+    const bool on = r < NP && flag[r] != 0;
+    const unsigned long long m = __builtin_amdgcn_ballot_w64(on);
+    if (on) live[(long)b * NP + n + __builtin_popcountll(m & ((1ull << lane) - 1ull))] = r;
+    n += __builtin_popcountll(m);
+  }
+  if (lane == 0) count[b] = n;
+}
+int launch_live_rows(const int32_t* nbr, int B, int NP, int NL, int K, const int32_t* np_real, const int32_t* nl_real, int32_t* live,
+                     int32_t* count, hipStream_t st) {
+  if (NP + NL > DD_N_MAX) return DD_ERR_UNSUPPORTED_SHAPE;
+  hipLaunchKernelGGL(k_live_rows, dim3(B), dim3(256), 0, st, nbr, B, NP, NL, K, np_real, nl_real, live, count);
+  DD_CHECK_LAUNCH();
+  return DD_OK;
+}
 int launch_layer0_rows(const float* tables, const int32_t* lig_v, const float* lig_aux, const int32_t* bond, int B, int NP, int NL,
                        float* l0_P, float* PL, float* l0_qn, float* qlnb, float* PB, float* qb, hipStream_t st) {
   const long atom_f4 = (long)B * NL * (160 + 320 + 32 + 32), bond_f4 = (long)B * NL * (NL - 1) * (160 + 32);
diff --git a/decompdiff_amd/csrc/dd_kernels.hpp b/decompdiff_amd/csrc/dd_kernels.hpp
--- a/decompdiff_amd/csrc/dd_kernels.hpp
+++ b/decompdiff_amd/csrc/dd_kernels.hpp
@@ -86,6 +86,8 @@
                     float* l0_P, float* PL, float* l0_qn, float* qlnb, float* PB, float* qb, hipStream_t st, int parts = 3,
                     int nv = DD_NUM_V);
 int launch_extract_ligand(const float* x, int B, int NP, int NL, float* out, hipStream_t st);
+int launch_live_rows(const int32_t* nbr, int B, int NP, int NL, int K, const int32_t* np_real, const int32_t* nl_real, int32_t* live,
+                     int32_t* count, hipStream_t st);
 
 enum { M_NE = 0, M_NB = 1, M_BL = 2, M_PE = 3, M_PB = 4 };
 
@@ -119,7 +121,9 @@
 };
 
 int launch_attn2(int mode, const AttnArgs& a, hipStream_t st);
-int launch_attn2_node(const AttnArgs& ne, const AttnArgs& nb, const AttnArgs& bl, hipStream_t st);
+int launch_attn2_node(const AttnArgs& ne, const AttnArgs& nb, const AttnArgs& bl, hipStream_t st, const int32_t* live = nullptr,
+                      const int32_t* live_count = nullptr);
+bool attn2_node_prunes(int NL);
 int launch_attn2_pos(const AttnArgs& pe, const AttnArgs& pb, hipStream_t st);
 int launch_attn2_pos_g(const AttnArgs& pe, const AttnArgs& pb, const GemmArgs* jobs, int njobs, int n_lead, int32_t* counter,
                        hipStream_t st);
diff --git a/decompdiff_amd/hip_lib.py b/decompdiff_amd/hip_lib.py
--- a/decompdiff_amd/hip_lib.py
+++ b/decompdiff_amd/hip_lib.py
@@ -25,7 +25,7 @@
 ]
 DEBUG_SYMBOLS = [
     "dd_workspace_view", "dd_profile_step", "dd_debug_set_clock_buffer", "dd_debug_set_fusion", "dd_debug_set_option",
-    "dd_debug_node_split", "dd_debug_node_split_cache_path", "dd_debug_schedule", "dd_debug_philox", "dd_debug_options_epoch", "dd_queue_error",
+    "dd_debug_node_split", "dd_debug_node_split_kind", "dd_debug_node_split_cache_path", "dd_debug_schedule", "dd_debug_philox", "dd_debug_options_epoch", "dd_queue_error",
 ]
 MEASUREMENT_ONLY_SYMBOLS = ("dd_queue_error",)
 BUILD_DEBUG_OPTIONS, BUILD_EXACT_MATH = 1, 2
@@ -71,7 +71,8 @@
 
 class DDWsView(ctypes.Structure):
     _fields_ = [("x", c_void_p), ("h", c_void_p), ("hb", c_void_p), ("ew", c_void_p), ("A", c_void_p),
-                ("nbr", c_void_p), ("Anb", c_void_p), ("lin_in_node", ctypes.c_int32)]
+                ("nbr", c_void_p), ("Anb", c_void_p), ("lin_in_node", ctypes.c_int32),
+                ("live", c_void_p), ("live_count", c_void_p)]
 
 
 PROF_CATS = ["misc", "gemm", "assemble", "attn_NE", "attn_NB", "attn_BL", "attn_PE", "attn_PB", "step", "event_pair"]
@@ -154,6 +155,7 @@
         "dd_debug_set_fusion": [c_int],
         "dd_debug_set_option": [c_int, c_int],
         "dd_debug_node_split": [c_int, c_int, c_int, c_int],
+        "dd_debug_node_split_kind": [c_int, c_int, c_int, c_int, c_int],
         "dd_debug_node_split_cache_path": [c_char_p, c_int],
         "dd_debug_schedule": [],
         "dd_reverse_step": [S, c_void_p, c_void_p, c_void_p, c_void_p],
diff --git a/include/decompdiff_hip_debug.h b/include/decompdiff_hip_debug.h
--- a/include/decompdiff_hip_debug.h
+++ b/include/decompdiff_hip_debug.h
@@ -20,6 +20,7 @@
 int dd_debug_set_option(int key, int value);
 int dd_debug_options_epoch(void);
 int dd_debug_node_split(int B, int NP, int NL, int K);
+int dd_debug_node_split_kind(int B, int NP, int NL, int K, int kind);
 int dd_debug_node_split_cache_path(char* out, int cap);
 int dd_debug_schedule(void);
 #if defined(DD_DEBUG_OPTIONS) && DD_DEBUG_OPTIONS
@@ -33,6 +34,8 @@
   int32_t* nbr;
   float* Anb;
   int32_t lin_in_node;
+  int32_t* live;
+  int32_t* live_count;
 } dd_ws_view;
 int dd_workspace_view(const dd_sampler* s, dd_ws_view* out);
 
```

After: 893.2 (median of 4 runs). No clear change (+0.9%).
